# zhaoyuhsin/Edge-Guided-Near-Eye-Image-Analysis-for-Head-Mounted-Displays

Measured on AMD Instinct MI355X. Metric: eye-frames/sec (320x240): inference edge+seg (value), +fit, exact fp32, and train fwd+bwd at 1 MI355X, higher is better.
Workload: dtype f32 tensors; inference products split into f16 hi/lo pairs (3 f16 MFMAs per product, 22-bit significand), f32 accumulate (`exact_fp32`: every product on the f32 MFMA); `train`: bf16 storage, f32 accumulate, f32 master weights (and an f32-storage leg)

## Files before the change

edge-guided-near-eye-image-analysis-for-head-mounted-displays_amd/bdcn_new.py:

```python
import ctypes as C

import torch
import torch.nn as nn

from . import _lib
from . import engine
from .engine import ACT_RELU, ConvLayer, Piece, PlanarPiece, Plan, VersionGuard, maxpool_out, pad8, require_cuda

import os
import types

PLANAR_IN = os.environ.get("EGNE_PLANAR_IN", "1") != "0"
SCORES_FUSED = os.environ.get("EGNE_SCORES_FUSED", "1") != "0"
MS_SIDE_STREAM = os.environ.get("EGNE_MS_SIDE", "1") != "0"
MS_SIDE_MIN_B = int(os.environ.get("EGNE_MS_SIDE_MIN_B", "8"))

_VGG = [("conv1_1", 3, 64, 1), ("conv1_2", 64, 64, 1), ("P", 2),
        ("conv2_1", 64, 128, 1), ("conv2_2", 128, 128, 1), ("P", 2),
        ("conv3_1", 128, 256, 1), ("conv3_2", 256, 256, 1), ("conv3_3", 256, 256, 1), ("P", 2),
        ("conv4_1", 256, 512, 1), ("conv4_2", 512, 512, 1), ("conv4_3", 512, 512, 1), ("P", 1),
        ("conv5_1", 512, 512, 2), ("conv5_2", 512, 512, 2), ("conv5_3", 512, 512, 2)]
_STAGES = [("1", ["1_1", "1_2"], 64), ("2", ["2_1", "2_2"], 128), ("3", ["3_1", "3_2", "3_3"], 256),
           ("4", ["4_1", "4_2", "4_3"], 512), ("5", ["5_1", "5_2", "5_3"], 512)]
_UPS = {"2": ("upsample_2", 2, 1), "3": ("upsample_4", 4, 2), "4": ("upsample_8", 8, 4), "5": ("upsample_8_5", 8, 0)}


def get_upsampling_weight(in_channels, out_channels, kernel_size):
    factor = (kernel_size + 1) // 2
    center = factor - 1 if kernel_size % 2 == 1 else factor - 0.5
    r = 1 - (torch.arange(kernel_size, dtype=torch.float64) - center).abs() / factor
    filt = r[:, None] * r[None, :]
    w = torch.zeros((in_channels, out_channels, kernel_size, kernel_size), dtype=torch.float64)
    for i in range(min(in_channels, out_channels)):
        w[i, i] = filt
    return w.float()


class VGG16_C(nn.Module):

    def __init__(self, pretrain=None, logger=None):
        super().__init__()
        for item in _VGG:
            if item[0] == "P":
                continue
            name, cin, cout, d = item
            conv = nn.Conv2d(cin, cout, 3, stride=1, padding=d, dilation=d)
            n = 9 * cout
            conv.weight.data.normal_(0, (2.0 / n) ** 0.5)
            conv.bias.data.zero_()
            setattr(self, name, conv)
        if pretrain:
            sd = torch.load(pretrain, map_location="cpu")
            own = self.state_dict()
            for k in own:
                if k in sd:
                    own[k].copy_(sd[k])


class MSBlock(nn.Module):

    def __init__(self, c_in, rate=4):
        super().__init__()
        self.rate = rate
        self.conv = nn.Conv2d(c_in, 32, 3, stride=1, padding=1)
        for i in (1, 2, 3):
            d = rate * i if rate >= 1 else 1
            setattr(self, "conv%d" % i, nn.Conv2d(32, 32, 3, stride=1, dilation=d, padding=d))
        for m in (self.conv, self.conv1, self.conv2, self.conv3):
            m.weight.data.normal_(0, 0.01)
            m.bias.data.zero_()


class BDCN(nn.Module):
    def __init__(self, pretrain=None, logger=None, rate=4):
        super().__init__()
        self.pretrain = pretrain
        self.rate = rate
        self.features = VGG16_C(pretrain, logger)
        for st, blocks, cin in _STAGES:
            for b in blocks:
                setattr(self, "msblock" + b, MSBlock(cin, rate))
                setattr(self, "conv%s_down" % b, nn.Conv2d(32, 21, (1, 1), stride=1))
            setattr(self, "score_dsn" + st, nn.Conv2d(21, 1, (1, 1), stride=1))
            setattr(self, "score_dsn%s_1" % st, nn.Conv2d(21, 1, (1, 1), stride=1))
        self.upsample_2 = nn.ConvTranspose2d(1, 1, 4, stride=2, bias=False)
        self.upsample_4 = nn.ConvTranspose2d(1, 1, 8, stride=4, bias=False)
        self.upsample_8 = nn.ConvTranspose2d(1, 1, 16, stride=8, bias=False)
        self.upsample_8_5 = nn.ConvTranspose2d(1, 1, 16, stride=8, bias=False)
        self.fuse = nn.Conv2d(10, 1, 1, stride=1)
        self._initialize_weights()
        self._plans = {}
        self.f16_products = 0
        self._events = None
        self.edge_thres = 0

    def _initialize_weights(self, logger=None):
        with torch.no_grad():
            for name, p in self.state_dict().items():
                if self.pretrain and "features" in name:
                    continue
                if "upsample" in name:
                    k = int(name.split(".")[0].split("_")[1])
                    p.copy_(get_upsampling_weight(1, 1, k * 2))
                elif "fuse" in name:
                    p.zero_() if "bias" in name else p.fill_(0.080)
                elif "bias" in name:
                    p.zero_()
                else:
                    p.normal_(0, 0.01)

    def _build(self, B, H, W, dev, only_fuse, edge_thres, f16_storage=None, split3=False):
        if f16_storage is None:
            h8, w8 = (maxpool_out(maxpool_out(maxpool_out(n, 2), 2), 2) for n in (H, W))
            if engine.PRESPLIT_TRUNK and engine.CALIBRATE and getattr(self, "_plan_products", 0) != 1 and B * h8 * w8 >= 256 * 128:
                try:
                    return self._build(B, H, W, dev, only_fuse, edge_thres, 0, True)
                except engine.NeedsFp32Storage:
                    pass
            if engine.F16_STORAGE and getattr(self, "_plan_products", 0) == 1:
                for level in ((2, 1) if engine.F16_STORAGE_DEEP else (1,)):
                    try:
                        return self._build(B, H, W, dev, only_fuse, edge_thres, level)
                    except engine.NeedsFp32Storage:
                        pass
            return self._build(B, H, W, dev, only_fuse, edge_thres, 0)
        pl = Plan(dev)
        pl.f16_storage = int(f16_storage)
        pl.split3_trunk = bool(split3)
        pl.f16_products = getattr(self, "_plan_products", 0)
        L = pl.L
        f = self.features
        x_in = pl.vec(B, 3, H, W)
        if PLANAR_IN and engine.F16X3_ENABLED and engine.C4H_MODE != "off":
            cur = PlanarPiece(x_in)
        else:
            xb = pl.buf(B, H, W, 8)
            pl.raw(L.egne_nchw_to_nhwc, (x_in.data_ptr(), B, 3, H, W, xb.data_ptr(), 8, 0, 8), "bdcn.in")
            cur = Piece(xb, 0, 3)
        ch, hh, ww = 3, H, W
        tail = _lib.BdcnTailDesc()
        tail.B, tail.H, tail.W = B, H, W
        block_of = {}
        for si, (st, blocks, cin) in enumerate(_STAGES):
            for bi, b in enumerate(blocks):
                block_of["conv" + b] = (si, bi)
        stages = {}
        side = MS_SIDE_STREAM and B >= MS_SIDE_MIN_B

        def stage_state(si, h_s, w_s):
            if si in stages:
                return stages[si]
            st, blocks, cin = _STAGES[si]
            nb = len(blocks)
            S = types.SimpleNamespace(st=st, blocks=blocks, nb=nb, h=h_s, w=w_s, ms_bufs=[], fused=None)
            S.o_buf = pl.buf(B, h_s, w_s, 32)
            S.dn = [getattr(self, "conv%s_down" % b) for b in blocks]
            S.sa, S.sb = getattr(self, "score_dsn" + st), getattr(self, "score_dsn%s_1" % st)
            S.s, S.s1 = pl.vec(B, h_s, w_s), pl.vec(B, h_s, w_s)
            S.cw, S.cc = pl.vec(nb, 2, 32), pl.vec(2)

            def refresh_scores(cw=S.cw, cc=S.cc, dn=S.dn, sa=S.sa, sb=S.sb):
                with torch.no_grad():
                    heads = torch.stack([sa.weight.detach().reshape(21), sb.weight.detach().reshape(21)])
                    for k, m in enumerate(dn):
                        cw[k].copy_(heads @ m.weight.detach().reshape(21, 32))
                    bsum = torch.stack([m.bias.detach() for m in dn]).sum(0)
                    cc.copy_(heads @ bsum + torch.cat([sa.bias.detach(), sb.bias.detach()]))
            S.refresh_scores = refresh_scores
            stages[si] = S
            return S

        def emit_block(si, bi, src, c_in, hh, ww):
            S = stage_state(si, hh, ww)
            b = S.blocks[bi]
            pl.side_default = side
            mb = getattr(self, "msblock" + b)
            l0 = ConvLayer([mb.conv.weight], [mb.conv.bias], [(c_in, pad8(c_in))], pad=(1, 1), act=ACT_RELU)
            l0.split = True
            o = Piece(S.o_buf, 0, 32)
            r = self.rate
            dil = tuple(r * i if r >= 1 else 1 for i in (1, 2, 3))
            lg = ConvLayer([mb.conv1.weight, mb.conv2.weight, mb.conv3.weight],
                           [mb.conv1.bias, mb.conv2.bias, mb.conv3.bias], [(32, 32)], pad=(1, 1), dils=dil,
                           act=ACT_RELU)
            lg.split = True
            if engine.PRESPLIT and pl.msdil_ok(lg, o, hh, ww):
                o.presplit = engine.SplitScale()
            pl.conv(l0, [src], o, B, hh, ww, name="ms%s.conv" % b)
            if not pl.last_presplit:
                o.presplit = None
            if S.fused is None:
                S.fused = SCORES_FUSED and pl.msdil_ok(lg, o, hh, ww)
                if S.fused:
                    pl.pre.append(VersionGuard([p for m in S.dn + [S.sa, S.sb] for p in (m.weight, m.bias)], S.refresh_scores))
            if S.fused:
                pl.conv(lg, [o], Piece(S.o_buf, 0, 32), B, hh, ww, residual=o, name="ms%s.dil" % b, scores=(S.cw[bi], S.cc, S.s, S.s1, bi > 0))
            else:
                msb = pl.buf(B, hh, ww, 32)
                pl.conv(lg, [o], Piece(msb, 0, 32), B, hh, ww, residual=o, name="ms%s.dil" % b)
                S.ms_bufs.append(msb)
            if bi == S.nb - 1:
                finish_stage(si, S)
            pl.side_default = False

        def finish_stage(si, S):
            st, nb, dn, sa, sb, s, s1 = S.st, S.nb, S.dn, S.sa, S.sb, S.s, S.s1
            if not S.fused:
                wd, bd = pl.vec(nb, 21, 32), pl.vec(nb, 21)
                heads = pl.vec(2, 21)
                hb = pl.vec(2)

                def refresh(wd=wd, bd=bd, heads=heads, hb=hb, dn=dn, sa=sa, sb=sb):
                    with torch.no_grad():
                        for k, m in enumerate(dn):
                            wd[k].copy_(m.weight.detach().reshape(21, 32))
                            bd[k].copy_(m.bias.detach())
                        heads[0].copy_(sa.weight.detach().reshape(21))
                        heads[1].copy_(sb.weight.detach().reshape(21))
                        hb[0:1].copy_(sa.bias.detach())
                        hb[1:2].copy_(sb.bias.detach())
                pl.pre.append(VersionGuard([p for m in dn + [sa, sb] for p in (m.weight, m.bias)], refresh))
                arr = (C.c_void_p * nb)(*[t.data_ptr() for t in S.ms_bufs])
                pl.keep.append(arr)
                pl.raw(L.egne_bdcn_stage_scores,
                       (arr, nb, 32, B * S.h * S.w, wd.data_ptr(), bd.data_ptr(), heads.data_ptr(), hb.data_ptr(),
                        heads.data_ptr() + 4 * 21, hb.data_ptr() + 4, s.data_ptr(), s1.data_ptr()), "bdcn.scores" + st)
            tail.s[si], tail.s1[si] = s.data_ptr(), s1.data_ptr()
            tail.h[si], tail.w[si] = S.h, S.w
            if st in _UPS:
                key, stride, crop = _UPS[st]
                upw = pl.vec(2 * stride, 2 * stride)
                mod = getattr(self, key)
                pl.pre.append(VersionGuard([mod.weight], lambda upw=upw, mod=mod: upw.copy_(
                    mod.weight.detach().reshape(upw.shape))))
                tail.up[si], tail.stride[si], tail.crop[si] = upw.data_ptr(), stride, crop
            else:
                tail.stride[si], tail.crop[si] = 1, 0

        pooled = None
        for idx, item in enumerate(_VGG):
            if item[0] == "P":
                s = item[1]
                ho, wo = maxpool_out(hh, s), maxpool_out(ww, s)
                if pooled is not None:
                    dst = pooled
                else:
                    c16 = getattr(cur, "f16s", None)
                    ob = (pl.buf16 if c16 is not None else pl.buf)(B, ho, wo, cur.Cp)
                    dst = Piece(ob, 0, cur.C)
                    dst.f16s = c16
                    dst.split3 = cur.split3
                    pl.maxpool2(cur, dst, B, hh, ww, s, "vgg.pool")
                cur, hh, ww, pooled = dst, ho, wo, None
                continue
            name, cin, cout, d = item
            conv = getattr(f, name)
            layer = ConvLayer([conv.weight], [conv.bias], [(cin, pad8(cin))], pad=(1, 1), dils=(d,), act=ACT_RELU)
            layer.split = cin % 32 == 0
            layer.split_c4 = cin <= 4
            h16 = (f16_storage >= 1 and name in ("conv1_1", "conv1_2")) or (f16_storage >= 2 and name[4] in "345")
            ob = (pl.buf16 if h16 else pl.buf)(B, hh, ww, cout)
            dst = Piece(ob, 0, cout)
            if h16:
                dst.f16s = engine.SplitScale()
            if split3 and name[4] in "345":
                dst.split3 = engine.SplitScale()
            nxt = _VGG[idx + 1] if idx + 1 < len(_VGG) else None
            pq = None
            if nxt is not None and nxt[0] == "P" and nxt[1] == 2:
                pq = Piece((pl.buf16 if h16 else pl.buf)(B, maxpool_out(hh, 2), maxpool_out(ww, 2), pad8(cout)), 0, cout)
                pq.f16s = dst.f16s
            pl.conv(layer, [cur], dst, B, hh, ww, name="vgg." + name, pool=pq)
            pooled = pq if pl.last_pooled else None
            cur = dst
            si, bi = block_of[name]
            emit_block(si, bi, dst, cout, hh, ww)
        pl.serial_timing = True
        pl.join_before.add(len(pl.calls))
        fw, fb = pl.vec(10), pl.vec(1)
        pl.pre.append(VersionGuard([self.fuse.weight, self.fuse.bias], lambda: (
            fw.copy_(self.fuse.weight.detach().reshape(10)), fb.copy_(self.fuse.bias.detach()))))
        tail.fuse_w, tail.fuse_b = fw.data_ptr(), fb.data_ptr()
        outs = pl.vec(11, B, 1, H, W)
        for k in range(11):
            tail.out[k] = outs[k].data_ptr() if (k == 10 or not only_fuse) else None
        tail.edge_thres = int(edge_thres)
        pl.keep.append(tail)
        pl.raw(L.egne_bdcn_tail, (C.byref(tail),), "bdcn.tail")
        pl.x_in, pl.outs = x_in, outs
        return pl

    def _plan(self, x, only_fuse, edge_thres=0):
        require_cuda(x, "BDCN input")
        for p in self.parameters():
            require_cuda(p, "BDCN parameters (call .cuda())")
            break
        B, Cc, H, W = x.shape
        if Cc != 3:
            raise ValueError("BDCN expects a 3-channel input, got %d" % Cc)
        prod = 1 if int(getattr(self, "f16_products", 0)) == 1 else 0
        key = (B, H, W, x.device, bool(only_fuse), int(edge_thres), prod)
        if key not in self._plans:
            self._plan_products = prod
            self._plans[key] = self._build(B, H, W, x.device, only_fuse, edge_thres)
        return self._plans[key]

    def forward(self, x):
        pl = self._plan(x, only_fuse=False)
        self._last_plan = pl
        pl.x_in.copy_(x.to(torch.float32))
        pl.run()
        return [pl.outs[k].clone() for k in range(11)]

    def forward_fuse(self, x, edge_thres=0):
        pl = self._plan(x, only_fuse=True, edge_thres=edge_thres)
        self._last_plan = pl
        pl.x_in.copy_(x.to(torch.float32))
        pl.run(self._events)
        return pl.outs[10].clone()

    def overflowed(self):
        pl = getattr(self, "_last_plan", None)
        return pl is not None and pl.overflowed()
```

edge-guided-near-eye-image-analysis-for-head-mounted-displays_amd/csrc/conv3x3_c4_f16.hip:

```cpp
#include "common.h"
#include "kernel_util.h"
#include "split_f16.h"

namespace {

__device__ __forceinline__ void split8(const u32x4 a, const u32x4 b, float s, h8& hi, h8& lo) {
  const f32x4 va = __builtin_bit_cast(f32x4, a), vb = __builtin_bit_cast(f32x4, b);
  const float x[8] = {va[0], va[1], va[2], va[3], vb[0], vb[1], vb[2], vb[3]};
#pragma unroll
  for (int q = 0; q < 4; ++q) {
    h2 h, l;
    egne::split2(x[2 * q], x[2 * q + 1], s, h, l);
    hi[2 * q] = h[0]; hi[2 * q + 1] = h[1];
    lo[2 * q] = l[0]; lo[2 * q + 1] = l[1];
  }
}

template <int TN>
__global__ __launch_bounds__(256) void conv3x3_c4_f16_kernel(const egne_conv_desc p, const _Float16* __restrict__ fhi,
                                                             const _Float16* __restrict__ flo, float a_scale, float out_scale,
                                                             long long M, int nblocks) {
  const int tid = threadIdx.x, lane = tid & 63, wave = tid >> 6;
  const int li = lane & 31, kq = lane >> 5;
  const egne_seg sg = p.seg[0];
  h8 wh[3][TN], wl[3][TN];
#pragma unroll
  for (int s = 0; s < 3; ++s)
#pragma unroll
    for (int tn = 0; tn < TN; ++tn) {
      wh[s][tn] = *(const h8*)(fhi + ((s * TN + tn) * 64 + lane) * 8);
      wl[s][tn] = *(const h8*)(flo + ((s * TN + tn) * 64 + lane) * 8);
    }
  const float slope = p.act == EGNE_ACT_RELU ? 0.f : (p.act == EGNE_ACT_LEAKY ? 0.01f : 1.f);
  f32x4 bias[TN][4], ps[TN][4], pt[TN][4];
#pragma unroll
  for (int tn = 0; tn < TN; ++tn)
#pragma unroll
    for (int j = 0; j < 4; ++j) {
      const int n = tn * 32 + 8 * j + 4 * kq;
      const bool nok = n < p.Cout_store;
      bias[tn][j] = (p.bias && nok) ? *(const f32x4*)(p.bias + n) : (f32x4)(0.f);
      ps[tn][j] = (p.post_scale && nok) ? *(const f32x4*)(p.post_scale + n) : (f32x4)(1.f);
      pt[tn][j] = (p.post_scale && nok) ? *(const f32x4*)(p.post_shift + n) : (f32x4)(0.f);
    }
  const int hw = p.H * p.W;
  const int ps4 = (int)sg.pix_stride * 4;
  const unsigned frame_in = (unsigned)hw * (unsigned)ps4;

  for (int blk = blockIdx.x * 4 + wave; blk < nblocks; blk += gridDim.x * 4) {
    const long long m = (long long)blk * 32 + li;
    const int b = (int)(m / hw);
    const int r = (int)(m - (long long)b * hw);
    const int y = r / p.W, x = r - y * p.W;
    const int b0 = (int)(((long long)blk * 32) / hw);
    const bool planar = sg.pix_stride == 1;
    const int fstride = planar ? hw * sg.Cp : hw * (int)sg.pix_stride;
    const long long left = ((long long)p.B - b0) * fstride * 4;
    const __amdgpu_buffer_rsrc_t rin = make_rsrc(sg.ptr + (long long)b0 * fstride, (unsigned)(left < 0x7fffffffll ? left : 0x7fffffffll));
    const int base = planar ? ((b - b0) * fstride + r) * 4 : (((b - b0) * hw + r) * (int)sg.pix_stride + sg.ch_off) * 4;
    (void)frame_in;
    f32x16 acc[TN];
#pragma unroll
    for (int tn = 0; tn < TN; ++tn) acc[tn] = (f32x16)(0.f);
    u32x4 xa[3], xb[3];
#pragma unroll
    for (int s = 0; s < 3; ++s) {
      const int t0 = 4 * s + 2 * kq, t1 = t0 + 1;
      const int dy0 = t0 / 3 - 1, dx0 = t0 % 3 - 1, dy1 = t1 / 3 - 1, dx1 = t1 % 3 - 1;
      const bool ok0 = m < M && t0 < 9 && (unsigned)(y + dy0) < (unsigned)p.H && (unsigned)(x + dx0) < (unsigned)p.W;
      const bool ok1 = m < M && t1 < 9 && (unsigned)(y + dy1) < (unsigned)p.H && (unsigned)(x + dx1) < (unsigned)p.W;
      if (planar) {
        const int o0 = ok0 ? base + (dy0 * p.W + dx0) * 4 : (int)OOB, o1 = ok1 ? base + (dy1 * p.W + dx1) * 4 : (int)OOB;
        u32x4 a = {0u, 0u, 0u, 0u}, c = {0u, 0u, 0u, 0u};
#pragma unroll
        for (int ch = 0; ch < 4; ++ch)
          if (ch < sg.Cp) {
            a[ch] = __builtin_amdgcn_raw_buffer_load_b32(rin, o0, ch * hw * 4, 0);
            c[ch] = __builtin_amdgcn_raw_buffer_load_b32(rin, o1, ch * hw * 4, 0);
          }
        xa[s] = a; xb[s] = c;
      } else {
        xa[s] = __builtin_amdgcn_raw_buffer_load_b128(rin, ok0 ? base + (dy0 * p.W + dx0) * ps4 : (int)OOB, 0, 0);
        xb[s] = __builtin_amdgcn_raw_buffer_load_b128(rin, ok1 ? base + (dy1 * p.W + dx1) * ps4 : (int)OOB, 0, 0);
      }
    }
#pragma unroll
    for (int s = 0; s < 3; ++s) {
      h8 ah, al;
      split8(xa[s], xb[s], a_scale, ah, al);
#pragma unroll
      for (int tn = 0; tn < TN; ++tn) {
        acc[tn] = __builtin_amdgcn_mfma_f32_32x32x16_f16(wh[s][tn], al, acc[tn], 0, 0, 0);
        acc[tn] = __builtin_amdgcn_mfma_f32_32x32x16_f16(wl[s][tn], ah, acc[tn], 0, 0, 0);
        acc[tn] = __builtin_amdgcn_mfma_f32_32x32x16_f16(wh[s][tn], ah, acc[tn], 0, 0, 0);
      }
    }
    const long long m0 = (long long)blk * 32;
    const long long rows = M - m0 < 32 ? M - m0 : 32;
    const bool o16 = p.out_split == 2;
    const int oesz = o16 ? 2 : 4;
    const __amdgpu_buffer_rsrc_t ro = make_rsrc((char*)p.out + m0 * p.out_pix_stride * oesz, (unsigned)(rows * p.out_pix_stride * oesz));
    bool bad = false;
#pragma unroll
    for (int tn = 0; tn < TN; ++tn)
#pragma unroll
      for (int j = 0; j < 4; ++j) {
        const int n = tn * 32 + 8 * j + 4 * kq;
        f32x4 v;
#pragma unroll
        for (int e = 0; e < 4; ++e) {
          const float t = acc[tn][4 * j + e] * out_scale + bias[tn][j][e];
          v[e] = fmaxf(t, t * slope) * ps[tn][j][e] + pt[tn][j][e];
        }
        if (tn == 0 && j == 0) bad |= egne_nonfinite(v[0]);
        if (o16) {
          const f32x2 u0 = {v[0] * p.out_split_scale, v[1] * p.out_split_scale}, u1 = {v[2] * p.out_split_scale, v[3] * p.out_split_scale};
          const h2 h0 = __builtin_convertvector(u0, h2), h1 = __builtin_convertvector(u1, h2);
          if (tn == 0 && j == 0) bad |= egne_nonfinite((float)h0[0]);
          const u32x2 two = {__builtin_bit_cast(unsigned, h0), __builtin_bit_cast(unsigned, h1)};
          __builtin_amdgcn_raw_buffer_store_b64(two, ro, n < p.Cout_store ? (li * (int)p.out_pix_stride + p.out_ch_off + n) * 2 : (int)OOB, 0, 0);
        } else
        __builtin_amdgcn_raw_buffer_store_b128(__builtin_bit_cast(u32x4, v), ro,
                                               n < p.Cout_store ? (li * (int)p.out_pix_stride + p.out_ch_off + n) * 4 : (int)OOB, 0, 0);
      }
    egne_ovf_commit(bad, p.ovf_flag);
  }
}

__global__ void pack_c4_f16_k(const float* __restrict__ w, int Cout, int Cin, int NT, float wscale, _Float16* __restrict__ hi,
                              _Float16* __restrict__ lo) {
  const int total = 3 * NT * 512;
  for (int i = blockIdx.x * blockDim.x + threadIdx.x; i < total; i += gridDim.x * blockDim.x) {
    const int j = i & 7, nn = (i >> 3) & 31, h = (i >> 8) & 1;
    const int q = i >> 9;
    const int tn = q % NT, s = q / NT;
    const int n = tn * 32 + nn, tap = 4 * s + 2 * h + (j >> 2), c = j & 3;
    const float v = (n < Cout && tap < 9 && c < Cin) ? w[((long long)n * Cin + c) * 9 + tap] * wscale : 0.f;
    const _Float16 hh = (_Float16)v;
    hi[i] = hh;
    lo[i] = (_Float16)(v - (float)hh);
  }
}

}

extern "C" int egne_pack_conv3x3_c4_weight_f16(const float* w_oihw, int Cout, int Cin, int CoutP, float wscale, void* fhi, void* flo,
                                               void* stream) {
  EGNE_REQUIRE(w_oihw && fhi && flo && Cout > 0 && Cin > 0 && Cin <= 4 && (CoutP == 32 || CoutP == 64) && Cout <= CoutP && wscale > 0.f,
               "pack_conv3x3_c4_f16: bad sizes Cout %d Cin %d CoutP %d", Cout, Cin, CoutP);
  hipLaunchKernelGGL(pack_c4_f16_k, dim3(6), dim3(256), 0, (hipStream_t)stream, w_oihw, Cout, Cin, CoutP / 32, wscale, (_Float16*)fhi,
                     (_Float16*)flo);
  return egne::check_launch("egne_pack_conv3x3_c4_weight_f16");
}

extern "C" int egne_conv3x3_smallcin_f16_fwd(const egne_conv_desc* dp, const void* fhi, const void* flo, float a_scale, float w_scale,
                                             void* stream) {
  EGNE_REQUIRE(dp && fhi && flo, "conv_smallcin_f16: null pointer");
  const egne_conv_desc& d = *dp;
  EGNE_REQUIRE(d.kh == 3 && d.kw == 3 && d.stride == 1 && d.pad_h == 1 && d.pad_w == 1 && d.pad_mode == 0 && d.ngroups == 1 &&
               d.dil[0] == 1 && d.nseg == 1 && d.Ho == d.H && d.Wo == d.W && !d.residual, "conv_smallcin_f16: geometry not supported");
  const egne_seg& g = d.seg[0];
  const bool planar = g.pix_stride == 1;
  EGNE_REQUIRE(g.ptr && !g.scale && ((uintptr_t)g.ptr & 15) == 0 &&
               (planar ? (g.Cp >= 1 && g.Cp <= 4 && g.ch_off == 0 && 2ll * d.H * d.W * g.Cp * 4 < (1ll << 31))
                       : (g.Cp >= 4 && g.ch_off % 4 == 0 && g.pix_stride % 4 == 0 && 2ll * d.H * d.W * g.pix_stride * 4 < (1ll << 31))),
               "conv_smallcin_f16: input slice");
  EGNE_REQUIRE((d.CoutP == 32 || d.CoutP == 64) && d.Cout_store <= d.CoutP && d.Cout_store % 4 == 0 && d.out && ((uintptr_t)d.out & 15) == 0 &&
               d.out_ch_off % 4 == 0 && d.out_pix_stride % 4 == 0 && d.out_ch_off + d.Cout_store <= d.out_pix_stride &&
               d.out_pix_stride * 128 < (1ll << 31) && (!d.bias || ((uintptr_t)d.bias & 15) == 0) &&
               (!d.post_scale || (((uintptr_t)d.post_scale & 15) == 0 && ((uintptr_t)d.post_shift & 15) == 0)), "conv_smallcin_f16: output");
  EGNE_REQUIRE(((uintptr_t)fhi & 15) == 0 && ((uintptr_t)flo & 15) == 0 && a_scale > 0.f && w_scale > 0.f, "conv_smallcin_f16: weights / scales");
  EGNE_REQUIRE(d.out_split == 0 || (d.out_split == 2 && d.out_split_scale > 0.f && !d.post_scale), "conv_smallcin_f16: f16 output (out_split = 2) needs a positive scale and no post affine");
  const long long M = (long long)d.B * d.H * d.W;
  const long long nb = (M + 31) / 32;
  EGNE_REQUIRE(nb < (1ll << 31), "conv_smallcin_f16: too many pixels");
  long long gx = (nb + 3) / 4;
  if (gx > 256 * 8) gx = 256 * 8;
  const float os = 1.0f / (a_scale * w_scale);
  hipStream_t st = (hipStream_t)stream;
  if (d.CoutP == 32)
    hipLaunchKernelGGL((conv3x3_c4_f16_kernel<1>), dim3((unsigned)gx), dim3(256), 0, st, d, (const _Float16*)fhi, (const _Float16*)flo, a_scale, os,
                       M, (int)nb);
  else
    hipLaunchKernelGGL((conv3x3_c4_f16_kernel<2>), dim3((unsigned)gx), dim3(256), 0, st, d, (const _Float16*)fhi, (const _Float16*)flo, a_scale, os,
                       M, (int)nb);
  return egne::check_launch("egne_conv3x3_smallcin_f16_fwd");
}
```

edge-guided-near-eye-image-analysis-for-head-mounted-displays_amd/csrc/conv3x3_rw_f16.hip:

```cpp
#include "common.h"
#include "kernel_util.h"
#include "split_f16.h"
#include <cstdlib>
#include <type_traits>

namespace {
__device__ int g_wdbg = 0;
__device__ unsigned long long g_wstamps[256 * 8 * 4];

constexpr int TW = 32, TH = 8, HWd = TW + 2, HHd = TH + 2, NPX = HHd * HWd;
constexpr int IMGH = 2 * NPX * 32;
constexpr int WCH = 9 * 2 * 2 * 512;
constexpr int NI = (NPX * 8 + 255) / 256;

template <int KCH, int NP = 3, bool F16IN = false, int SH = 0>
__global__ __launch_bounds__(512)
void conv3x3_rw_kernel(const egne_conv_desc p, const _Float16* __restrict__ fhi, const _Float16* __restrict__ flo, float a_scale,
                       float out_scale, int tiles_x, int tiles_y, int ntiles, int ncb, int nrun) {
  egne::dyn_scales(p.dyn_scale, a_scale, out_scale);
  extern __shared__ __attribute__((aligned(16))) _Float16 ldsh[];
  _Float16* const lw = ldsh + 2 * IMGH;

  const int dbg = g_wdbg;
  unsigned long long t_work = 0, t_wait = 0, t_hand = 0, t_last = 0;
  auto stamp = [&](unsigned long long& accum) {
    if (dbg & 64) {
      asm volatile("s_waitcnt lgkmcnt(0)" ::: "memory");
      const unsigned long long t = __builtin_amdgcn_s_memtime();
      accum += t - t_last; t_last = t;
    }
  };
  const int tid = threadIdx.x, lane = tid & 63;
  const int wave = __builtin_amdgcn_readfirstlane(tid >> 6);
  const int li = lane & 31, lh = lane >> 5;
  const int H = p.H, W = p.W;
  const egne_seg sg = p.seg[0];

  const int xcd = blockIdx.x & 7, q = blockIdx.x >> 3;
  const int wpx = ((int)gridDim.x >> 3) / nrun;
  if (q >= wpx * nrun) return;
  const int cb = q % nrun, worker = (q / nrun) * 8 + xcd, nworkers = wpx * 8;
  auto tile_at = [&](int i) { return worker + i * nworkers; };
  struct Tile { int b, y0, x0; };
  auto decode = [&](int t) {
    Tile r;
    const int tx = t % tiles_x; t /= tiles_x;
    const int ty = t % tiles_y; t /= tiles_y;
    r.b = t; r.y0 = ty * TH; r.x0 = tx * TW;
    return r;
  };
  int ntl = 0;
  while (tile_at(ntl) < ntiles) ++ntl;
  constexpr bool STREAM = KCH == 0;
  const int nk = STREAM ? p.Ktot / 32 : KCH;
  const int nmine = ntl * nk;
  const int nloop = (nmine + 1) & ~1;

  const int KT16 = nk * 2;
  if constexpr (!STREAM) {
    for (int it = tid; it < KCH * 9 * 2 * 2 * 64; it += 512) {
      const int l = it & 63, hl = (it >> 6) & 1, ks = (it >> 7) & 1, r = it >> 8, tap = r % 9, ch = r / 9;
      const long long src = (((long long)tap * KT16 + ch * 2 + ks) * ncb + cb) * 512 + l * 8;
      *(u32x4*)&lw[(long long)it * 8] = *(const u32x4*)((hl ? flo : fhi) + src);
    }
  }
  __syncthreads();

  if (wave < 4) {
    constexpr int NPC = F16IN ? 4 : 8, PGS = 256 / NPC, CPP = 32 / NPC, ESZ = F16IN ? 2 : 4, NQ = (NPX * NPC + 255) / 256;
    const int piece = tid & (NPC - 1), pg = tid / NPC;
    const float slope_in = sg.act_in == EGNE_ACT_RELU ? 0.f : (sg.act_in == EGNE_ACT_LEAKY ? 0.01f : 1.f);
    const int lofs = F16IN ? pg * 32 + ((piece ^ ((pg >> 1) & 3)) << 3) : pg * 32 + (((piece >> 1) ^ ((pg >> 1) & 3)) << 3) + ((piece & 1) << 2);
    u32x4 st[2][NQ];
    int rel[NQ];
#pragma unroll
    for (int I = 0; I < NQ; ++I) {
      const int px = pg + PGS * I, hy = px / HWd, hx = px - hy * HWd;
      rel[I] = px < NPX ? (((hy - 1) * W + hx - 1) * (int)sg.pix_stride + sg.ch_off + piece * CPP) * ESZ : (int)OOB;
    }
    struct Job { Tile t; int ch; };
    auto job_at = [&](int j) { Job r; r.t = decode(tile_at(j / nk)); r.ch = j % nk; return r; };
    auto issue1 = [&](const Job& jb, bool on, auto bc, auto ic) {
      constexpr int BUF = decltype(bc)::value, I = decltype(ic)::value;
      const Tile& tl = jb.t;
      const __amdgpu_buffer_rsrc_t r = make_rsrc((const char*)sg.ptr + (long long)tl.b * H * W * sg.pix_stride * ESZ, (unsigned)H * W * (unsigned)sg.pix_stride * (unsigned)ESZ);
      const int c0 = jb.ch * 32 + piece * CPP;
      int off;
      if (tl.x0 >= 1 && tl.x0 + TW + 1 <= W) {
        const int sbase = ((tl.y0 * W + tl.x0) * (int)sg.pix_stride + jb.ch * 32) * ESZ;
        off = (on && c0 < sg.Cp && rel[I] != (int)OOB) ? rel[I] + sbase : (int)OOB;
      } else {
        int pq = pg;
        asm volatile("" : "+v"(pq));
        const int px = pq + PGS * I;
        const int hy = px / HWd, hx = px - hy * HWd;
        const int y = tl.y0 - 1 + hy, x = tl.x0 - 1 + hx;
        const bool ok = on && c0 < sg.Cp && px < NPX && (unsigned)y < (unsigned)H && (unsigned)x < (unsigned)W;
        off = ok ? ((y * W + x) * (int)sg.pix_stride + sg.ch_off + c0) * ESZ : (int)OOB;
      }
      st[BUF][I] = __builtin_amdgcn_raw_buffer_load_b128(r, off, 0, 0);
    };
    f32x4 asc[2] = {{1.f, 1.f, 1.f, 1.f}, {1.f, 1.f, 1.f, 1.f}}, ash[2] = {{0.f, 0.f, 0.f, 0.f}, {0.f, 0.f, 0.f, 0.f}};
    auto load_aff = [&](const Job& jb, auto bc) {
      constexpr int BUF = decltype(bc)::value;
      if (sg.scale && nmine > 0) {
        const int c0 = jb.ch * 32 + piece * 4;
        const float* zs = c0 < sg.Cp ? sg.scale + (long long)jb.t.b * sg.Cp + c0 : egne_zero_page;
        const float* zh = c0 < sg.Cp ? sg.shift + (long long)jb.t.b * sg.Cp + c0 : egne_zero_page;
        asc[BUF] = *(const f32x4*)zs;
        ash[BUF] = *(const f32x4*)zh;
      }
    };
    auto convert1 = [&](const Job& jb, _Float16* img, auto bc, auto ic) {
      constexpr int BUF = decltype(bc)::value, I = decltype(ic)::value;
      const int px = pg + PGS * I;
      if constexpr (F16IN) {
        if (I < NQ - 1 || px < NPX) *(u32x4*)&img[lofs + 32 * PGS * I] = st[BUF][I];
        return;
      }
      if (I < NQ - 1 || px < NPX) {
        f32x4 v = __builtin_bit_cast(f32x4, st[BUF][I]);
        if (sg.scale) {
          const int hy = px / HWd, hx = px - hy * HWd;
          const int y = jb.t.y0 - 1 + hy, x = jb.t.x0 - 1 + hx;
#pragma unroll
          for (int e = 0; e < 4; ++e) {
            const float t = v[e] * asc[BUF][e] + ash[BUF][e];
            v[e] = fmaxf(t, t * slope_in);
          }
          if (!((unsigned)y < (unsigned)H && (unsigned)x < (unsigned)W)) v = (f32x4)(0.f);
        }
        const int o = lofs + 32 * PGS * I;
        if constexpr (NP == 1) {
          float t0, t1, t2, t3;
          asm("v_mul_f32_e32 %0, %1, %2" : "=v"(t0) : "s"(a_scale), "v"(v[0]));
          asm("v_mul_f32_e32 %0, %1, %2" : "=v"(t1) : "s"(a_scale), "v"(v[1]));
          asm("v_mul_f32_e32 %0, %1, %2" : "=v"(t2) : "s"(a_scale), "v"(v[2]));
          asm("v_mul_f32_e32 %0, %1, %2" : "=v"(t3) : "s"(a_scale), "v"(v[3]));
          const egne::sp_f32x2 u0 = {t0, t1}, u1 = {t2, t3};
          const h2 h0 = __builtin_convertvector(u0, h2), h1 = __builtin_convertvector(u1, h2);
          const h4 hi = {h0[0], h0[1], h1[0], h1[1]};
          *(h4*)&img[o] = hi;
        } else {
        h2 h0, h1, l0, l1;
        egne::split2(v[0], v[1], a_scale, h0, l0);
        egne::split2(v[2], v[3], a_scale, h1, l1);
        const h4 hi = {h0[0], h0[1], h1[0], h1[1]}, lo = {l0[0], l0[1], l1[0], l1[1]};
        *(h4*)&img[o] = hi;
        *(h4*)&img[NPX * 32 + o] = lo;
        }
      }
    };
    u32x4 wreg[STREAM ? 9 : 1];
    const unsigned wbytes = 9u * (unsigned)KT16 * (unsigned)ncb * 1024u;
    const __amdgpu_buffer_rsrc_t rwh = make_rsrc(fhi, wbytes), rwl = make_rsrc(flo, wbytes);
    auto w_issue = [&](int ch, bool on) {
#pragma unroll
      for (int i = 0; i < (STREAM ? 9 : 0); ++i) {
        const int it = tid + 256 * i, l = it & 63, hl = (it >> 6) & 1, ks = (it >> 7) & 1, tap = it >> 8;
        const int off = on ? ((((tap * KT16 + ch * 2 + ks) * ncb + cb) * 512 + l * 8) * 2) : (int)OOB;
        wreg[i] = hl ? __builtin_amdgcn_raw_buffer_load_b128(rwl, off, 0, 0) : __builtin_amdgcn_raw_buffer_load_b128(rwh, off, 0, 0);
      }
    };
    auto w_store = [&](int parity) {
#pragma unroll
      for (int i = 0; i < (STREAM ? 9 : 0); ++i) *(u32x4*)&lw[parity * WCH + (tid + 256 * i) * 8] = wreg[i];
    };
    auto step = [&](int s, auto bc) {
      constexpr int BUF = decltype(bc)::value;
      const bool c_on = s + 1 < nmine, i_on = s + 3 < nmine;
      const Job jc = job_at(c_on ? s + 1 : 0), ji = job_at(i_on ? s + 3 : 0);
      if constexpr (STREAM) {
        w_store((s + 1) & 1);
        w_issue(job_at(s + 2 < nmine ? s + 2 : 0).ch, s + 2 < nmine);
      }
      load_aff(job_at(s + 2 < nmine ? s + 2 : 0), std::integral_constant<int, BUF ^ 1>{});
      _Float16* img = ldsh + ((s + 1) & 1) * IMGH;
      [&]<int... Is>(std::integer_sequence<int, Is...>) {
        (([&] {
          if (c_on) convert1(jc, img, bc, std::integral_constant<int, Is>{});
          issue1(ji, i_on, bc, std::integral_constant<int, Is>{});
        }()), ...);
      }(std::make_integer_sequence<int, NQ>{});
    };
    using B0 = std::integral_constant<int, 0>;
    using B1 = std::integral_constant<int, 1>;
    {
      const Job j0 = job_at(0), j1 = job_at(nmine > 1 ? 1 : 0), j2 = job_at(nmine > 2 ? 2 : 0);
      if constexpr (STREAM) {
        w_issue(j0.ch, nmine > 0);
        w_store(0);
        w_issue(j1.ch, nmine > 1);
      }
      load_aff(j0, B0{});
      load_aff(j1, B1{});
      [&]<int... Is>(std::integer_sequence<int, Is...>) {
        (issue1(j0, nmine > 0, B0{}, std::integral_constant<int, Is>{}), ...);
        (issue1(j1, nmine > 1, B1{}, std::integral_constant<int, Is>{}), ...);
      }(std::make_integer_sequence<int, NQ>{});
      [&]<int... Is>(std::integer_sequence<int, Is...>) {
        (([&] {
          if (nmine > 0) convert1(j0, ldsh, B0{}, std::integral_constant<int, Is>{});
          issue1(j2, nmine > 2, B0{}, std::integral_constant<int, Is>{});
        }()), ...);
      }(std::make_integer_sequence<int, NQ>{});
    }
    lds_barrier();
    t_last = __builtin_amdgcn_s_memtime();
    for (int s = 0; s < nloop; s += 2) {
      step(s, B1{});
      stamp(t_work); lds_barrier(); stamp(t_wait);
      step(s + 1, B0{});
      stamp(t_work); lds_barrier(); stamp(t_wait);
    }
  } else if constexpr (SH != 0) {
    constexpr bool GEN = SH == 1;
    const int cw = wave - 4, row0 = cw * 2;
    const int l15 = lane & 15, kg = lane >> 4;
    const bool o16 = GEN && NP == 1 && p.out_split == 2;
    const bool split_on = SH == 4 || (GEN && !o16 && p.out_split != 0);
    const bool pool_on = SH == 3 || (GEN && p.pool_out != nullptr);
    const bool full_epi = SH == 5 || (GEN && (p.post_scale != nullptr || p.residual != nullptr));
    const int oesz = o16 ? 2 : 4;
    const unsigned frame_out = (unsigned)H * W * (unsigned)p.out_pix_stride * (unsigned)oesz;
    const unsigned frame_res = (unsigned)H * W * (unsigned)p.res_pix_stride * 4u;
    const int Hp = (H + 1) >> 1, Wp = (W + 1) >> 1;
    const unsigned frame_pool = (unsigned)Hp * Wp * (unsigned)p.pool_pix_stride * (unsigned)oesz;
    const float slope_out = p.act == EGNE_ACT_RELU ? 0.f : (p.act == EGNE_ACT_LEAKY ? 0.01f : 1.f);
    f32x4 b4[2];
    bool jok[2];
#pragma unroll
    for (int nh = 0; nh < 2; ++nh) {
      const int n = cb * 32 + nh * 16 + 4 * kg;
      b4[nh] = p.bias ? *(const f32x4*)(p.bias + n) : (f32x4)(0.f);
      jok[nh] = n < p.Cout_store;
    }
    int aofs[9][2][2];
#pragma unroll
    for (int tap = 0; tap < 9; ++tap)
#pragma unroll
      for (int tm = 0; tm < 2; ++tm)
#pragma unroll
        for (int ph = 0; ph < 2; ++ph) {
          const int qq = (row0 + tm + tap / 3) * HWd + ph * 16 + l15 + tap % 3;
          aofs[tap][tm][ph] = qq * 32 + ((kg ^ ((qq >> 1) & 3)) << 3);
        }
    const int wl = (kg >> 1) * 1024 + ((kg & 1) * 32 + l15) * 8;
    int xl[2], xlp[2], lco[2], lcr[2], lcp[2];
#pragma unroll
    for (int ph = 0; ph < 2; ++ph) {
      xl[ph] = ph * 16 + l15;
      xlp[ph] = (l15 & 1) ? 0x40000000 : xl[ph];
      lco[ph] = (xl[ph] * (int)p.out_pix_stride + p.out_ch_off + cb * 32 + 4 * kg) * oesz;
      lcr[ph] = (xl[ph] * (int)p.res_pix_stride + p.res_ch_off + cb * 32 + 4 * kg) * 4;
      lcp[ph] = ((xl[ph] >> 1) * (int)p.pool_pix_stride + p.pool_ch_off + cb * 32 + 4 * kg) * oesz;
    }
    f32x4 R[2][2][2][2];
#pragma unroll
    for (int a = 0; a < 16; ++a) (&R[0][0][0][0])[a] = (f32x4)(0.f);
    __amdgpu_buffer_rsrc_t rout = make_rsrc(p.out, 0u), rres = make_rsrc(nullptr, 0u), rpo = make_rsrc(nullptr, 0u);
    int wlim[2] = {0, 0}, sbo[2] = {0, 0}, sbr[2] = {0, 0}, wlim_p = 0, x1lim = 0, sbp = 0;
    bool y1 = false;
    bool have_prev = false;
    unsigned ovf_m = 0u, ovf_h = 0u;
    int tvo = (int)OOB, tvr = (int)OOB, poff = (int)OOB;
    auto epi = [&](auto qc, auto gc) {
      constexpr int Q = decltype(qc)::value, Gi = decltype(gc)::value, nh = Gi & 1, ph = (Gi >> 1) & 1, tm = Gi >> 2;
      if constexpr (tm == 0) {
        if (pool_on) {
          const bool x1 = xl[ph] < x1lim;
          if constexpr (nh == 0) poff = xlp[ph] < wlim_p ? lcp[ph] + sbp : (int)OOB;
          f32x4 v;
#pragma unroll
          for (int e = 0; e < 4; ++e) {
            float m = R[Q][0][ph][nh][e];
            m = y1 ? fmaxf(m, R[Q][1][ph][nh][e]) : m;
            const float qn = __builtin_bit_cast(float, __builtin_amdgcn_update_dpp(0, __builtin_bit_cast(int, m), 0xB1, 0xf, 0xf, false));
            m = x1 ? fmaxf(m, qn) : m;
            const float t = m * out_scale + b4[nh][e];
            v[e] = fmaxf(t, t * slope_out);
          }
          if (o16) {
            const egne::sp_f32x2 u0 = {v[0] * p.out_split_scale, v[1] * p.out_split_scale}, u1 = {v[2] * p.out_split_scale, v[3] * p.out_split_scale};
            const h2 h0 = __builtin_convertvector(u0, h2), h1 = __builtin_convertvector(u1, h2);
            const u32x2 two = {__builtin_bit_cast(unsigned, h0), __builtin_bit_cast(unsigned, h1)};
            __builtin_amdgcn_raw_buffer_store_b64(two, rpo, jok[nh] ? poff : (int)OOB, nh * 32, 0);
          } else {
            __builtin_amdgcn_raw_buffer_store_b128(__builtin_bit_cast(u32x4, v), rpo, jok[nh] ? poff : (int)OOB, nh * 64, 0);
          }
        }
      }
      if constexpr (nh == 0) {
        const bool okp = xl[ph] < wlim[tm];
        tvo = okp ? lco[ph] + sbo[tm] : (int)OOB;
        if (full_epi) tvr = okp ? lcr[ph] + sbr[tm] : (int)OOB;
      }
      f32x4 v;
#pragma unroll
      for (int e = 0; e < 4; ++e) {
        const float t = R[Q][tm][ph][nh][e] * out_scale + b4[nh][e];
        v[e] = fmaxf(t, t * slope_out);
      }
      if (full_epi) {
        const int n = cb * 32 + nh * 16 + 4 * kg;
        if (p.post_scale) {
          const f32x4 ps = *(const f32x4*)(p.post_scale + n), pt = *(const f32x4*)(p.post_shift + n);
#pragma unroll
          for (int e = 0; e < 4; ++e) v[e] = v[e] * ps[e] + pt[e];
        }
        if (p.residual) {
          const f32x4 rv = __builtin_bit_cast(f32x4, __builtin_amdgcn_raw_buffer_load_b128(rres, jok[nh] ? tvr : (int)OOB, nh * 64, 0));
#pragma unroll
          for (int e = 0; e < 4; ++e) v[e] += rv[e];
        }
      }
      if constexpr (nh == 0) ovf_m = max(ovf_m, __builtin_bit_cast(unsigned, v[0]) & 0x7fffffffu);
      if (o16) {
        const egne::sp_f32x2 u0 = {v[0] * p.out_split_scale, v[1] * p.out_split_scale}, u1 = {v[2] * p.out_split_scale, v[3] * p.out_split_scale};
        const h2 h0 = __builtin_convertvector(u0, h2), h1 = __builtin_convertvector(u1, h2);
        if constexpr (nh == 0) ovf_h = max(ovf_h, __builtin_bit_cast(unsigned, h0) & 0x7fffu);
        const u32x2 two = {__builtin_bit_cast(unsigned, h0), __builtin_bit_cast(unsigned, h1)};
        __builtin_amdgcn_raw_buffer_store_b64(two, rout, jok[nh] ? tvo : (int)OOB, nh * 32, 0);
      } else if (split_on) {
        h2 h0, h1, l0, l1;
        egne::split2(v[0], v[1], p.out_split_scale, h0, l0);
        egne::split2(v[2], v[3], p.out_split_scale, h1, l1);
        const u32x4 pk = {__builtin_bit_cast(unsigned, h0), __builtin_bit_cast(unsigned, h1), __builtin_bit_cast(unsigned, l0), __builtin_bit_cast(unsigned, l1)};
        R[Q][tm][ph][nh] = __builtin_bit_cast(f32x4, pk);
        if constexpr (nh == 1) {
          const u32x4 p0 = __builtin_bit_cast(u32x4, R[Q][tm][ph][0]), p1 = __builtin_bit_cast(u32x4, R[Q][tm][ph][1]);
          const u32x4 hi = {p0[0], p0[1], p1[0], p1[1]}, lo = {p0[2], p0[3], p1[2], p1[3]};
          __builtin_amdgcn_raw_buffer_store_b128(hi, rout, tvo, 0, 0);
          if constexpr (NP == 3) __builtin_amdgcn_raw_buffer_store_b128(lo, rout, tvo, 64, 0);
        }
      } else {
        __builtin_amdgcn_raw_buffer_store_b128(__builtin_bit_cast(u32x4, v), rout, jok[nh] ? tvo : (int)OOB, nh * 64, 0);
      }
    };
    const int d_tx = nworkers % tiles_x, d_ty = (nworkers / tiles_x) % tiles_y, d_b = (nworkers / tiles_x) / tiles_y;
    int tx = worker % tiles_x, ty = (worker / tiles_x) % tiles_y, tb = (worker / tiles_x) / tiles_y;
    int s = 0;
    auto job = [&](auto pc, auto fc, int ch) {
      constexpr int P = decltype(pc)::value;
      constexpr bool FIRST = decltype(fc)::value;
      const _Float16* Thi = ldsh + (s & 1) * IMGH;
      const _Float16* Tlo = Thi + NPX * 32;
      const _Float16* wb = lw + (STREAM ? (s & 1) : ch) * WCH + wl;
      h8 wh[2][2], wo[2][2], ah[2][2][2], al[2][2][2];
      auto fetch = [&](auto tc) {
        constexpr int T = decltype(tc)::value, Bq = T & 1;
#pragma unroll
        for (int nh = 0; nh < 2; ++nh) {
          wh[Bq][nh] = *(const h8*)&wb[T * 2048 + nh * 128];
          if constexpr (NP == 3) wo[Bq][nh] = *(const h8*)&wb[T * 2048 + 512 + nh * 128];
        }
#pragma unroll
        for (int tm = 0; tm < 2; ++tm)
#pragma unroll
          for (int ph = 0; ph < 2; ++ph) {
            ah[Bq][tm][ph] = *(const h8*)&Thi[aofs[T][tm][ph]];
            if constexpr (NP == 3) al[Bq][tm][ph] = *(const h8*)&Tlo[aofs[T][tm][ph]];
          }
      };
      fetch(std::integral_constant<int, 0>{});
      [&]<int... Ts>(std::integer_sequence<int, Ts...>) {
        (([&] {
          constexpr int t = Ts, Bq = t & 1;
          __builtin_amdgcn_sched_barrier(0);
          if constexpr (t + 1 < 9) fetch(std::integral_constant<int, t + 1>{});
          if constexpr (FIRST && t < 8) epi(std::integral_constant<int, P ^ 1>{}, std::integral_constant<int, t>{});
#pragma unroll
          for (int tm = 0; tm < 2; ++tm)
#pragma unroll
            for (int ph = 0; ph < 2; ++ph)
#pragma unroll
              for (int nh = 0; nh < 2; ++nh) {
                f32x4 c = R[P][tm][ph][nh];
                if constexpr (FIRST && t == 0) c = (f32x4)(0.f);
                if constexpr (NP == 3) {
                  c = __builtin_amdgcn_mfma_f32_16x16x32_f16(wh[Bq][nh], al[Bq][tm][ph], c, 0, 0, 0);
                  c = __builtin_amdgcn_mfma_f32_16x16x32_f16(wo[Bq][nh], ah[Bq][tm][ph], c, 0, 0, 0);
                }
                c = __builtin_amdgcn_mfma_f32_16x16x32_f16(wh[Bq][nh], ah[Bq][tm][ph], c, 0, 0, 0);
                R[P][tm][ph][nh] = c;
              }
          constexpr int NM = NP == 3 ? 24 : 8, ND = t + 1 < 9 ? (NP == 3 ? 12 : 6) : 0, NV = FIRST && SH == 3 && t < 4 ? 4 : 3;
          [&]<int... Ms>(std::integer_sequence<int, Ms...>) {
            (([&] {
              __builtin_amdgcn_sched_group_barrier(0x8, 1, 0);
              if constexpr (Ms < ND) __builtin_amdgcn_sched_group_barrier(0x100, 1, 0);
              __builtin_amdgcn_sched_group_barrier(0x2, NV, 0);
              if constexpr (FIRST && Ms >= NM - 3) __builtin_amdgcn_sched_group_barrier(0x40, 1, 0);
            }()), ...);
          }(std::make_integer_sequence<int, NM>{});
        }()), ...);
      }(std::make_integer_sequence<int, 9>{});
      __builtin_amdgcn_sched_barrier(0);
      ++s;
      stamp(t_work); lds_barrier(); stamp(t_wait);
    };
    auto tile = [&](auto pc) {
      job(pc, std::true_type{}, 0);
      for (int ch = 1; ch < nk; ++ch) job(pc, std::false_type{}, ch);
      const int py = ty * TH + row0, px = tx * TW;
#pragma unroll
      for (int tm = 0; tm < 2; ++tm) {
        const bool in = py + tm < H;
        wlim[tm] = in ? W - px : 0;
        sbo[tm] = in ? ((py + tm) * W + px) * (int)p.out_pix_stride * oesz : 0;
        if (full_epi) sbr[tm] = in ? ((py + tm) * W + px) * (int)p.res_pix_stride * 4 : 0;
      }
      if (pool_on) {
        y1 = py + 1 < H; x1lim = W - px - 1; wlim_p = wlim[0];
        sbp = py < H ? ((py >> 1) * Wp + (px >> 1)) * (int)p.pool_pix_stride * oesz : 0;
      }
      rout = make_rsrc((char*)p.out + (long long)tb * H * W * p.out_pix_stride * oesz, frame_out);
      if (full_epi) rres = make_rsrc(p.residual ? p.residual + (long long)tb * H * W * p.res_pix_stride : nullptr, p.residual ? frame_res : 0u);
      if (pool_on) rpo = make_rsrc((char*)p.pool_out + (long long)tb * Hp * Wp * p.pool_pix_stride * oesz, frame_pool);
      if (!have_prev) ovf_m = ovf_h = 0u;
      have_prev = true;
      tx += d_tx;
      int c = tx >= tiles_x ? 1 : 0;
      tx -= c ? tiles_x : 0;
      ty += d_ty + c;
      c = ty >= tiles_y ? 1 : 0;
      ty -= c ? tiles_y : 0;
      tb += d_b + c;
    };
    using P0 = std::integral_constant<int, 0>;
    using P1 = std::integral_constant<int, 1>;
    lds_barrier();
    t_last = __builtin_amdgcn_s_memtime();
    for (int i = 0; i < ntl; i += 2) {
      tile(P0{});
      if (i + 1 < ntl) tile(P1{});
    }
    if (nmine & 1) { stamp(t_work); lds_barrier(); stamp(t_wait); }
    stamp(t_work);
    if (have_prev) {
      auto flush = [&](auto qc) {
        [&]<int... Gs>(std::integer_sequence<int, Gs...>) { (epi(qc, std::integral_constant<int, Gs>{}), ...); }(std::make_integer_sequence<int, 8>{});
      };
      if (ntl & 1) flush(P0{}); else flush(P1{});
    }
    stamp(t_hand);
    const bool ovf_bad = egne_nonfinite(__builtin_bit_cast(float, ovf_m)) || egne_nonfinite((float)__builtin_bit_cast(_Float16, (unsigned short)ovf_h));
    egne_ovf_commit(ovf_bad, p.ovf_flag);
  } else {
    const int cw = wave - 4, row0 = cw * 2;
    const int l15 = lane & 15, kg = lane >> 4;
    const bool o16 = NP == 1 && p.out_split == 2;
    const int oesz = o16 ? 2 : 4;
    const unsigned frame_out = (unsigned)H * W * (unsigned)p.out_pix_stride * (unsigned)oesz;
    const unsigned frame_res = (unsigned)H * W * (unsigned)p.res_pix_stride * 4u;
    const float slope_out = p.act == EGNE_ACT_RELU ? 0.f : (p.act == EGNE_ACT_LEAKY ? 0.01f : 1.f);
    const bool full_epi = p.post_scale != nullptr || p.residual != nullptr;
    f32x4 b4[2];
    bool jok[2];
#pragma unroll
    for (int nh = 0; nh < 2; ++nh) {
      const int n = cb * 32 + nh * 16 + 4 * kg;
      b4[nh] = p.bias ? *(const f32x4*)(p.bias + n) : (f32x4)(0.f);
      jok[nh] = n < p.Cout_store;
    }
    int aofs[9][2][2];
#pragma unroll
    for (int tap = 0; tap < 9; ++tap)
#pragma unroll
      for (int tm = 0; tm < 2; ++tm)
#pragma unroll
        for (int ph = 0; ph < 2; ++ph) {
          const int qq = (row0 + tm + tap / 3) * HWd + ph * 16 + l15 + tap % 3;
          aofs[tap][tm][ph] = qq * 32 + ((kg ^ ((qq >> 1) & 3)) << 3);
        }
    const int wl = (kg >> 1) * 1024 + ((kg & 1) * 32 + l15) * 8;
    f32x4 acc[2][2][2], prev[2][2][2];
#pragma unroll
    for (int a = 0; a < 8; ++a) { (&acc[0][0][0])[a] = (f32x4)(0.f); (&prev[0][0][0])[a] = (f32x4)(0.f); }
    __amdgpu_buffer_rsrc_t rout = make_rsrc(p.out, 0u), rres = make_rsrc(nullptr, 0u);
    int tvo[2][2], tvr[2][2];
#pragma unroll
    for (int a = 0; a < 4; ++a) { (&tvo[0][0])[a] = (int)OOB; (&tvr[0][0])[a] = (int)OOB; }
    bool ovf_bad = false;
    auto finish_group = [&](auto gc) {
      constexpr int Gi = decltype(gc)::value, nh = Gi & 1, ph = (Gi >> 1) & 1, tm = Gi >> 2;
      f32x4 v;
#pragma unroll
      for (int e = 0; e < 4; ++e) {
        const float t = prev[tm][ph][nh][e] * out_scale + b4[nh][e];
        v[e] = fmaxf(t, t * slope_out);
      }
      if (full_epi) {
        const int n = cb * 32 + nh * 16 + 4 * kg;
        if (p.post_scale) {
          const f32x4 ps = *(const f32x4*)(p.post_scale + n), pt = *(const f32x4*)(p.post_shift + n);
#pragma unroll
          for (int e = 0; e < 4; ++e) v[e] = v[e] * ps[e] + pt[e];
        }
        if (p.residual) {
          const f32x4 rv = __builtin_bit_cast(f32x4, __builtin_amdgcn_raw_buffer_load_b128(rres, jok[nh] ? tvr[tm][ph] : (int)OOB, nh * 64, 0));
#pragma unroll
          for (int e = 0; e < 4; ++e) v[e] += rv[e];
        }
      }
      if constexpr (nh == 0) ovf_bad |= egne_nonfinite(v[0]);
      if (o16) {
        const egne::sp_f32x2 u0 = {v[0] * p.out_split_scale, v[1] * p.out_split_scale}, u1 = {v[2] * p.out_split_scale, v[3] * p.out_split_scale};
        const h2 h0 = __builtin_convertvector(u0, h2), h1 = __builtin_convertvector(u1, h2);
        if constexpr (nh == 0) ovf_bad |= egne_nonfinite((float)h0[0]);
        v[0] = __builtin_bit_cast(float, h0);
        v[1] = __builtin_bit_cast(float, h1);
      } else if (p.out_split) {
        h2 h0, h1, l0, l1;
        egne::split2(v[0], v[1], p.out_split_scale, h0, l0);
        egne::split2(v[2], v[3], p.out_split_scale, h1, l1);
        const u32x4 pk = {__builtin_bit_cast(unsigned, h0), __builtin_bit_cast(unsigned, h1), __builtin_bit_cast(unsigned, l0), __builtin_bit_cast(unsigned, l1)};
        v = __builtin_bit_cast(f32x4, pk);
      }
      prev[tm][ph][nh] = v;
    };
    auto store_group = [&](auto gc) {
      constexpr int Gi = decltype(gc)::value, nh = Gi & 1, ph = (Gi >> 1) & 1, tm = Gi >> 2;
      if (o16) {
        const u32x4 pk = __builtin_bit_cast(u32x4, prev[tm][ph][nh]);
        const u32x2 two = {pk[0], pk[1]};
        __builtin_amdgcn_raw_buffer_store_b64(two, rout, jok[nh] ? tvo[tm][ph] : (int)OOB, nh * 32, 0);
      } else if (p.out_split) {
        if constexpr (nh == 1) {
          const u32x4 p0 = __builtin_bit_cast(u32x4, prev[tm][ph][0]), p1 = __builtin_bit_cast(u32x4, prev[tm][ph][1]);
          const u32x4 hi = {p0[0], p0[1], p1[0], p1[1]}, lo = {p0[2], p0[3], p1[2], p1[3]};
          __builtin_amdgcn_raw_buffer_store_b128(hi, rout, tvo[tm][ph], 0, 0);
          if constexpr (NP == 3) __builtin_amdgcn_raw_buffer_store_b128(lo, rout, tvo[tm][ph], 64, 0);
        }
      } else {
        __builtin_amdgcn_raw_buffer_store_b128(__builtin_bit_cast(u32x4, prev[tm][ph][nh]), rout, jok[nh] ? tvo[tm][ph] : (int)OOB, nh * 64, 0);
      }
    };
    bool have_prev = false;
    lds_barrier();
    t_last = __builtin_amdgcn_s_memtime();
    for (int s = 0; s < nloop; ++s) {
      if (s < nmine) {
        const int ch = s % nk;
        const Tile tl = decode(tile_at(s / nk));
        const _Float16* Thi = ldsh + (s & 1) * IMGH;
        const _Float16* Tlo = Thi + NPX * 32;
        const _Float16* wb = lw + (STREAM ? (s & 1) : ch) * WCH + wl;
        if (ch == 0) {
#pragma unroll
          for (int a = 0; a < 8; ++a) (&acc[0][0][0])[a] = (f32x4)(0.f);
        }
        h8 wh[2][2], wo[2][2], ah[2][2][2], al[2][2][2];
        auto fetch = [&](auto tc) {
          constexpr int T = decltype(tc)::value, Bq = T & 1;
#pragma unroll
          for (int nh = 0; nh < 2; ++nh) {
            wh[Bq][nh] = *(const h8*)&wb[T * 2048 + nh * 128];
            if constexpr (NP == 3) wo[Bq][nh] = *(const h8*)&wb[T * 2048 + 512 + nh * 128];
          }
#pragma unroll
          for (int tm = 0; tm < 2; ++tm)
#pragma unroll
            for (int ph = 0; ph < 2; ++ph) {
              ah[Bq][tm][ph] = *(const h8*)&Thi[aofs[T][tm][ph]];
              if constexpr (NP == 3) al[Bq][tm][ph] = *(const h8*)&Tlo[aofs[T][tm][ph]];
            }
        };
        fetch(std::integral_constant<int, 0>{});
        [&]<int... Ts>(std::integer_sequence<int, Ts...>) {
          (([&] {
            constexpr int t = Ts, Bq = t & 1;
            if constexpr (t + 1 < 9) fetch(std::integral_constant<int, t + 1>{});
            if constexpr (t < 8) { if (ch == 0 && have_prev) store_group(std::integral_constant<int, t>{}); }
            __builtin_amdgcn_sched_barrier(0);
#pragma unroll
            for (int tm = 0; tm < 2; ++tm)
#pragma unroll
              for (int ph = 0; ph < 2; ++ph)
#pragma unroll
                for (int nh = 0; nh < 2; ++nh) {
                  f32x4& c = acc[tm][ph][nh];
                  if constexpr (NP == 3) {
                    c = __builtin_amdgcn_mfma_f32_16x16x32_f16(wh[Bq][nh], al[Bq][tm][ph], c, 0, 0, 0);
                    c = __builtin_amdgcn_mfma_f32_16x16x32_f16(wo[Bq][nh], ah[Bq][tm][ph], c, 0, 0, 0);
                  }
                  c = __builtin_amdgcn_mfma_f32_16x16x32_f16(wh[Bq][nh], ah[Bq][tm][ph], c, 0, 0, 0);
                }
            __builtin_amdgcn_sched_barrier(0);
          }()), ...);
        }(std::make_integer_sequence<int, 9>{});
        if (ch == nk - 1) {
          stamp(t_work);
          const int y = tl.y0 + row0;
          if (p.pool_out) {
            const int Hp = (H + 1) >> 1, Wp = (W + 1) >> 1;
            const __amdgpu_buffer_rsrc_t rpo = make_rsrc((char*)p.pool_out + (long long)tl.b * Hp * Wp * p.pool_pix_stride * oesz,
                                                         (unsigned)Hp * Wp * (unsigned)p.pool_pix_stride * (unsigned)oesz);
            const bool y1 = y + 1 < H;
#pragma unroll
            for (int ph = 0; ph < 2; ++ph) {
              const int x = tl.x0 + ph * 16 + l15;
              const bool x1 = x + 1 < W;
              const int poff = (!(l15 & 1) && x < W && y < H) ? (((y >> 1) * Wp + (x >> 1)) * (int)p.pool_pix_stride + p.pool_ch_off + cb * 32 + 4 * kg) * oesz : (int)OOB;
#pragma unroll
              for (int nh = 0; nh < 2; ++nh) {
                f32x4 v;
#pragma unroll
                for (int e = 0; e < 4; ++e) {
                  float m = acc[0][ph][nh][e];
                  if (y1) m = fmaxf(m, acc[1][ph][nh][e]);
                  const float qn = __builtin_bit_cast(float, __builtin_amdgcn_update_dpp(0, __builtin_bit_cast(int, m), 0xB1, 0xf, 0xf, false));
                  if (x1) m = fmaxf(m, qn);
                  const float t = m * out_scale + b4[nh][e];
                  v[e] = fmaxf(t, t * slope_out);
                }
                if (o16) {
                  const egne::sp_f32x2 u0 = {v[0] * p.out_split_scale, v[1] * p.out_split_scale}, u1 = {v[2] * p.out_split_scale, v[3] * p.out_split_scale};
                  const h2 h0 = __builtin_convertvector(u0, h2), h1 = __builtin_convertvector(u1, h2);
                  const u32x2 two = {__builtin_bit_cast(unsigned, h0), __builtin_bit_cast(unsigned, h1)};
                  __builtin_amdgcn_raw_buffer_store_b64(two, rpo, jok[nh] ? poff : (int)OOB, nh * 32, 0);
                } else {
                  __builtin_amdgcn_raw_buffer_store_b128(__builtin_bit_cast(u32x4, v), rpo, jok[nh] ? poff : (int)OOB, nh * 64, 0);
                }
              }
            }
          }
#pragma unroll
          for (int a = 0; a < 8; ++a) (&prev[0][0][0])[a] = (&acc[0][0][0])[a];
          rout = make_rsrc((char*)p.out + (long long)tl.b * H * W * p.out_pix_stride * oesz, frame_out);
          rres = make_rsrc(p.residual ? p.residual + (long long)tl.b * H * W * p.res_pix_stride : nullptr, p.residual ? frame_res : 0u);
#pragma unroll
          for (int tm = 0; tm < 2; ++tm)
#pragma unroll
            for (int ph = 0; ph < 2; ++ph) {
              const int yy = y + tm, x = tl.x0 + ph * 16 + l15;
              const bool okp = yy < H && x < W;
              tvo[tm][ph] = okp ? ((yy * W + x) * (int)p.out_pix_stride + p.out_ch_off + cb * 32 + 4 * kg) * oesz : (int)OOB;
              tvr[tm][ph] = okp ? ((yy * W + x) * (int)p.res_pix_stride + p.res_ch_off + cb * 32 + 4 * kg) * 4 : (int)OOB;
            }
          [&]<int... Gs>(std::integer_sequence<int, Gs...>) { (finish_group(std::integral_constant<int, Gs>{}), ...); }(std::make_integer_sequence<int, 8>{});
          have_prev = true;
          stamp(t_hand);
        }
      }
      stamp(t_work); lds_barrier(); stamp(t_wait);
    }
    if (have_prev)
      [&]<int... Gs>(std::integer_sequence<int, Gs...>) { (store_group(std::integral_constant<int, Gs>{}), ...); }(std::make_integer_sequence<int, 8>{});
    egne_ovf_commit(ovf_bad, p.ovf_flag);
  }
  if ((dbg & 64) && lane == 0) {
    unsigned long long* o = g_wstamps + ((long long)blockIdx.x * 8 + wave) * 4;
    o[0] = t_work + t_hand; o[1] = t_wait; o[2] = nmine; o[3] = t_hand;
  }
}

template <int KCH, int NP, bool F16IN, int SH>
int launch_rw_form(const egne_conv_desc& d, const _Float16* fhi, const _Float16* flo, float a_scale, float os, hipStream_t st);

template <int KCH, int NP = 3, bool F16IN = false>
int launch_rw(const egne_conv_desc& d, const _Float16* fhi, const _Float16* flo, float a_scale, float os, hipStream_t st) {
  const char* e = getenv("EGNE_RW_SHADOW");
  if (e && e[0] == '0') return launch_rw_form<KCH, NP, F16IN, 0>(d, fhi, flo, a_scale, os, st);
  if constexpr (NP == 3) {
    if ((d.post_scale || d.residual) && d.pool_out) return launch_rw_form<KCH, NP, F16IN, 0>(d, fhi, flo, a_scale, os, st);
    if (d.post_scale || d.residual) return launch_rw_form<KCH, NP, F16IN, 5>(d, fhi, flo, a_scale, os, st);
    if (d.pool_out) return launch_rw_form<KCH, NP, F16IN, 3>(d, fhi, flo, a_scale, os, st);
    if (d.out_split) return launch_rw_form<KCH, NP, F16IN, 4>(d, fhi, flo, a_scale, os, st);
    return launch_rw_form<KCH, NP, F16IN, 2>(d, fhi, flo, a_scale, os, st);
  } else {
    return launch_rw_form<KCH, NP, F16IN, 1>(d, fhi, flo, a_scale, os, st);
  }
}

template <int KCH, int NP, bool F16IN, int SH>
int launch_rw_form(const egne_conv_desc& d, const _Float16* fhi, const _Float16* flo, float a_scale, float os, hipStream_t st) {
  const int tiles_x = (d.W + TW - 1) / TW, tiles_y = (d.H + TH - 1) / TH;
  const int ntiles = tiles_x * tiles_y * d.B, ncb = d.CoutP / 32, nrun = (d.Cout_store + 31) / 32;
  constexpr size_t lds = ((size_t)2 * IMGH + (size_t)(KCH == 0 ? 2 : KCH) * WCH) * sizeof(_Float16);
  static_assert(lds <= 163840, "LDS budget");
  if (!egne::raise_lds((const void*)conv3x3_rw_kernel<KCH, NP, F16IN, SH>, lds)) return egne::fail(EGNE_ERR_LAUNCH, "conv3x3_rw: cannot raise the dynamic LDS limit to %zu", lds);
  hipLaunchKernelGGL((conv3x3_rw_kernel<KCH, NP, F16IN, SH>), dim3(256), dim3(512), lds, st, d, fhi, flo, a_scale, os, tiles_x, tiles_y, ntiles, ncb, nrun);
  return egne::check_launch("egne_conv3x3_rw_f16_fwd");
}

}

extern "C" int egne_conv3x3_rw_f16_fwd(const egne_conv_desc* dp, const void* fhi, const void* flo, float a_scale, float w_scale,
                                       void* stream) {
  EGNE_REQUIRE(dp && fhi && flo, "conv3x3_rw: null pointer");
  const egne_conv_desc& d = *dp;
  EGNE_REQUIRE(d.kh == 3 && d.kw == 3 && d.stride == 1 && d.pad_mode == 0 && d.ngroups == 1 && d.nseg == 1 && d.pad_h == 1 &&
               d.pad_w == 1 && d.dil[0] == 1 && d.Ho == d.H && d.Wo == d.W && !d.stats_ws, "conv3x3_rw: geometry / options not supported");
  const egne_seg& g = d.seg[0];
  EGNE_REQUIRE(g.ptr && g.Cp % 8 == 0 && (g.Cp + 31) / 32 * 32 == d.Ktot && d.Ktot >= 32 && d.Ktot <= 1024 && g.ch_off % 4 == 0 &&
               g.pix_stride % 4 == 0 && ((uintptr_t)g.ptr & 15) == 0 && (g.scale == nullptr) == (g.shift == nullptr), "conv3x3_rw: input slice");
  EGNE_REQUIRE(d.CoutP % 32 == 0 && d.CoutP <= 256 && d.Cout_store >= 8 && d.Cout_store <= d.CoutP && d.Cout_store % 8 == 0 && d.out &&
               ((uintptr_t)d.out & 15) == 0 && d.out_pix_stride % 4 == 0 && d.out_ch_off % 4 == 0 &&
               d.out_ch_off + d.Cout_store <= d.out_pix_stride && (!d.bias || ((uintptr_t)d.bias & 15) == 0), "conv3x3_rw: output");
  EGNE_REQUIRE(!d.residual || (((uintptr_t)d.residual & 15) == 0 && d.res_pix_stride % 4 == 0 && d.res_ch_off % 4 == 0), "conv3x3_rw: residual alignment");
  EGNE_REQUIRE(!d.post_scale || (((uintptr_t)d.post_scale & 15) == 0 && ((uintptr_t)d.post_shift & 15) == 0), "conv3x3_rw: post affine alignment");
  EGNE_REQUIRE(!d.pool_out || (((uintptr_t)d.pool_out & 15) == 0 && d.pool_pix_stride % 4 == 0 && d.pool_ch_off % 4 == 0 && !d.post_scale &&
                                d.pool_ch_off + d.Cout_store <= d.pool_pix_stride &&
                                (long long)((d.H + 1) / 2) * ((d.W + 1) / 2) * d.pool_pix_stride * 4 < (1ll << 31)), "conv3x3_rw: pooled output");
  EGNE_REQUIRE(((uintptr_t)fhi & 15) == 0 && ((uintptr_t)flo & 15) == 0 && a_scale > 0.f && w_scale > 0.f, "conv3x3_rw: weights / scales");
  EGNE_REQUIRE(d.out_split != 1 || (d.out_split_scale > 0.f && d.Cout_store % 32 == 0 && d.out_ch_off % 32 == 0 && !d.pool_out && !d.post_scale && !d.residual),
               "conv3x3_rw: split-pair output needs whole 32-channel blocks, a positive scale and no pooled / post-affine / residual options");
  EGNE_REQUIRE(d.out_split == 0 || d.out_split == 1 || (d.out_split == 2 && d.f16_products == 1 && d.out_split_scale > 0.f && !d.post_scale && !d.residual),
               "conv3x3_rw: f16 output (out_split = 2) needs f16_products = 1, a positive scale and no post-affine / residual options");
  const bool in16 = g.presplit == 2;
  EGNE_REQUIRE(g.presplit == 0 || (in16 && d.f16_products == 1 && !g.scale && g.ch_off % 8 == 0 && g.pix_stride % 8 == 0 &&
                                   (long long)d.H * d.W * g.pix_stride * 2 < (1ll << 31)),
               "conv3x3_rw: an f16 input slice (presplit = 2) needs f16_products = 1, no fused affine and 16-byte aligned pixels");
  EGNE_REQUIRE((long long)d.H * d.W * g.pix_stride * 4 < (1ll << 31) && (long long)d.H * d.W * d.out_pix_stride * 4 < (1ll << 31) &&
               (!d.residual || (long long)d.H * d.W * d.res_pix_stride * 4 < (1ll << 31)), "conv3x3_rw: frame too large for 32-bit byte offsets");
  const float os = 1.0f / (a_scale * w_scale);
  hipStream_t st = (hipStream_t)stream;
  const _Float16 *h = (const _Float16*)fhi, *l = (const _Float16*)flo;
  if (d.f16_products == 1 && in16) {
    if (d.Ktot == 32) return launch_rw<1, 1, true>(d, h, l, a_scale, os, st);
    if (d.Ktot == 64) return launch_rw<2, 1, true>(d, h, l, a_scale, os, st);
    return launch_rw<0, 1, true>(d, h, l, a_scale, os, st);
  }
  if (d.f16_products == 1) {
    if (d.Ktot == 32) return launch_rw<1, 1>(d, h, l, a_scale, os, st);
    if (d.Ktot == 64) return launch_rw<2, 1>(d, h, l, a_scale, os, st);
    return launch_rw<0, 1>(d, h, l, a_scale, os, st);
  }
  if (d.Ktot == 32) return launch_rw<1>(d, h, l, a_scale, os, st);
  if (d.Ktot == 64) return launch_rw<2>(d, h, l, a_scale, os, st);
  return launch_rw<0>(d, h, l, a_scale, os, st);
}

extern "C" int egne_rw_debug(int dbg, void* out_stamps) {
  if (hipMemcpyToSymbol(HIP_SYMBOL(g_wdbg), &dbg, sizeof(int)) != hipSuccess) return -2;
  if (out_stamps && hipMemcpyFromSymbol(out_stamps, HIP_SYMBOL(g_wstamps), sizeof(unsigned long long) * 256 * 8 * 4) != hipSuccess) return -2;
  return 0;
}
```

edge-guided-near-eye-image-analysis-for-head-mounted-displays_amd/engine.py:

```python
import collections
import ctypes as C
import types

import torch

from . import _lib
from ._lib import ACT_LEAKY, ACT_NONE, ACT_RELU


import os

HALO_ENABLED = os.environ.get("EGNE_HALO", "1") != "0"
F16X3_ENABLED = os.environ.get("EGNE_F16X3", "1") != "0"
HALO_F16_MAX_COUTP = int(os.environ.get("EGNE_HALO_F16_MAX_COUTP", "256"))
LATTICE_ENABLED = os.environ.get("EGNE_LATTICE", "1") != "0"
LAYER_BYTES = {}
TDPOOL_FUSED = os.environ.get("EGNE_TDPOOL_FUSED", "1") != "0"
TDPOOL_STATS_UNITS = 32768
HALO_POOL = os.environ.get("EGNE_HALO_POOL", "1") != "0"
POOL_FUSED = os.environ.get("EGNE_POOL_FUSED", "1") != "0"
RW_MIN_W = int(os.environ.get("EGNE_RW_MIN_W", "120"))
RW_MAX_COUTP = int(os.environ.get("EGNE_RW_MAX_COUTP", "32"))
RW_MAX_CP = int(os.environ.get("EGNE_RW_MAX_CP", "512"))
RW_ENABLED = os.environ.get("EGNE_RW", "1") != "0"
RS_ENABLED = os.environ.get("EGNE_RS", "1") != "0"
RS_MIN_W = int(os.environ.get("EGNE_RS_MIN_W", "60"))
RS_MIN_W_F16 = int(os.environ.get("EGNE_RS_MIN_W_F16", "30"))
RW_MIN_W_F16 = int(os.environ.get("EGNE_RW_MIN_W_F16", "30"))
NARROW_F32 = os.environ.get("EGNE_NARROW_F32", "1") != "0"
TAIL16_HALO = os.environ.get("EGNE_TAIL16_HALO", "1") != "0"
MSDIL_ENABLED = os.environ.get("EGNE_MSDIL", "1") != "0"
LATTICE_MIN_W = int(os.environ.get("EGNE_LATTICE_MIN_W", "20"))
S1X1_ENABLED = os.environ.get("EGNE_S1X1", "1") != "0"
MS1X1_ENABLED = os.environ.get("EGNE_MS1X1", "1") != "0"
C4H_MODE = os.environ.get("EGNE_C4H", "wide")
MS1X1_MIN_PIX = int(os.environ.get("EGNE_MS1X1_MIN_PIX", "30000"))
BIG_ENABLED = os.environ.get("EGNE_BIG", "1") != "0"
SMALL_ENABLED = os.environ.get("EGNE_SMALL", "1") != "0"
BIG_MIN_COUT = int(os.environ.get("EGNE_BIG_MIN_COUT", "256"))
BIG_MIN_CIN = int(os.environ.get("EGNE_BIG_MIN_CIN", "64"))
BIG_SPLIT_TAIL = os.environ.get("EGNE_BIG_SPLIT_TAIL", "1") != "0"
BIG_CUS = 256
BIG1_ENABLED = os.environ.get("EGNE_BIG1", "1") != "0"
WINDOW_NAME = os.environ.get("EGNE_FIT_WINDOW", "enc.b3.conv1")
WINDOW_HOOKS = []
EVENT_KINDS = None
S1X1_MIN_PIX = int(os.environ.get("EGNE_S1X1_MIN_PIX", "100000"))
HALO_F16_ENABLED = os.environ.get("EGNE_HALO_F16", "1") != "0"
ESF_SPLIT = os.environ.get("EGNE_ESF_SPLIT", "1") != "0"
ZERO_SKIP = os.environ.get("EGNE_ZERO_SKIP", "1") != "0"
FIRST_WRITER = os.environ.get("EGNE_FIRST_WRITER", "1") != "0"
PAIR_BIAS = os.environ.get("EGNE_PAIR_BIAS", "1") != "0"
ZERO_AHEAD = os.environ.get("EGNE_ZERO_AHEAD", "1") != "0"
PAIR_BIAS_SIDE = os.environ.get("EGNE_PAIR_BIAS_SIDE", "1") != "0"
MERGE_DGRAD = os.environ.get("EGNE_MERGE_DGRAD", "1") != "0"
WGRAD_SPLIT = os.environ.get("EGNE_WGRAD_SPLIT", "1") != "0"
WGRAD_SIDE_STREAM = os.environ.get("EGNE_WGRAD_SIDE", "1") != "0"
WSCALE_EVERY = int(os.environ.get("EGNE_WSCALE_EVERY", "16"))
TRAIN_SPLIT = os.environ.get("EGNE_TRAIN_SPLIT", "1") != "0"
F16X3_ASCALE = float(os.environ.get("EGNE_F16X3_ASCALE", "16"))
STATS_FUSED = os.environ.get("EGNE_STATS_FUSED", "1") != "0"
STATS_FUSED_BF16 = os.environ.get("EGNE_STATS_FUSED_BF16", "1") != "0"
FUSE_1X1 = os.environ.get("EGNE_FUSE_1X1", "1") != "0"
FUSE_1X1_MIN_W = int(os.environ.get("EGNE_FUSE_1X1_MIN_W", "60"))
FUSE_C4 = os.environ.get("EGNE_FUSE_C4", "1") != "0"
C1V = os.environ.get("EGNE_C1V", "1") != "0"
CALIBRATE = os.environ.get("EGNE_CALIBRATE", "1") != "0"
RECAL_EVERY = int(os.environ.get("EGNE_RECAL_EVERY", "1024"))
CHECK_DISPATCH = os.environ.get("EGNE_CHECK_DISPATCH", "0") != "0"
DISPATCH_LOG = []
OVF_CHECK = os.environ.get("EGNE_OVF_CHECK", "1") != "0"
SMALLCIN_ENABLED = os.environ.get("EGNE_SMALLCIN", "1") != "0"
HALO_MIN_W = int(os.environ.get("EGNE_HALO_MIN_W", "30"))
HALO_TALL = os.environ.get("EGNE_SHALO_TALL", "1") != "0"
HALO_F16_MIN_W = int(os.environ.get("EGNE_HALO_F16_MIN_W", "30"))
HALO_F16_MIN_W_NARROW = int(os.environ.get("EGNE_HALO_F16_MIN_W_NARROW", "30"))
HALO_MAX_COUTP = int(os.environ.get("EGNE_HALO_MAX_COUTP", "128"))
NORM_FUSE = os.environ.get("EGNE_NORM_FUSE", "1") != "0"
PREFIX_ACC = os.environ.get("EGNE_PREFIX_ACC", "1") != "0"
BN_ACT_FUSE = os.environ.get("EGNE_BN_ACT_FUSE", "1") != "0"
MULTI_DGRAD = os.environ.get("EGNE_MULTI_DGRAD", "1") != "0"
MASK_ON_WRITE = os.environ.get("EGNE_MASK_ON_WRITE", "1") != "0"
MULTI_SINGLE = os.environ.get("EGNE_MULTI_SINGLE", "1") != "0"
MASK3_ON_WRITE = os.environ.get("EGNE_MASK3_ON_WRITE", "1") != "0"
BF16_FAST1X1 = os.environ.get("EGNE_BF16_FAST1X1", "1") != "0"
BF16_DGRAD_PACK = os.environ.get("EGNE_BF16_DGRAD_PACK", "1") != "0"
BF16_NARROW = os.environ.get("EGNE_BF16_NARROW", "1") != "0"
BF16_FAST3X3 = os.environ.get("EGNE_BF16_FAST3X3", "1") != "0"


def pad8(c):
    return (int(c) + 7) // 8 * 8


def pad32(c):
    return (int(c) + 31) // 32 * 32


def _ptr(t, elem_off=0):
    return t.data_ptr() + 4 * int(elem_off)


class Piece:

    __slots__ = ("buf", "off", "C", "Cp", "n0", "scale", "shift", "act_in", "nograd", "presplit", "norm_fuse", "f16s", "split3")

    def __init__(self, buf, off, C_, Cp=None, n0=0):
        self.buf, self.off, self.C, self.Cp, self.n0 = buf, int(off), int(C_), int(Cp or pad8(C_)), int(n0)
        self.scale = self.shift = None
        self.act_in = ACT_NONE
        self.nograd = False
        self.presplit = None
        self.f16s = None
        self.split3 = None
        self.norm_fuse = False
        assert self.off % 4 == 0 and self.Cp % 8 == 0 and self.off + self.Cp <= buf.shape[-1]

    @property
    def stride(self):
        return self.buf.shape[-1]

    @property
    def ptr(self):
        hw = self.buf.shape[1] * self.buf.shape[2]
        return self.buf.data_ptr() + self.buf.element_size() * (self.n0 * hw * self.stride)

    def with_norm(self, scale, shift, act_in=ACT_NONE):
        p = Piece(self.buf, self.off, self.C, self.Cp, self.n0)
        p.scale, p.shift, p.act_in, p.nograd, p.norm_fuse = scale, shift, act_in, self.nograd, self.norm_fuse
        return p

    def samples(self, n0):
        return Piece(self.buf, self.off, self.C, self.Cp, n0)


class SplitScale:

    def __init__(self):
        self.value = F16X3_ASCALE


class NeedsFp32Storage(Exception):
    """Plan.conv: a slice held as f16 (Piece.f16s) met a kernel that neither writes nor reads that storage -- the plan builder falls
    back to fp32 tensors (bdcn_new.BDCN._build)."""


F16_STORAGE = os.environ.get("EGNE_F16_STORAGE", "1") != "0"
F16_STORAGE_DEEP = os.environ.get("EGNE_F16_STORAGE_DEEP", "1") != "0"
PRESPLIT_TRUNK = os.environ.get("EGNE_PRESPLIT_TRUNK", "1") != "0"
PRESPLIT = os.environ.get("EGNE_PRESPLIT", "1") != "0"
SPLIT_PAIR_PERM = torch.tensor([16 * ((p >> 2) & 1) + 4 * (p >> 3) + (p & 3) for p in range(32)])


class ConvLayer:

    def __init__(self, weights, biases, in_layout, stride=1, pad=(0, 0), dils=(1,), act=ACT_NONE, pad_mode=0,
                 kernel_hw=None, cout_pad=None):
        self.weights = list(weights)
        self.biases = list(biases) if biases is not None else None
        self.in_layout = [(int(c), int(cp)) for c, cp in in_layout]
        w0 = self.weights[0]
        self.Cout = w0.shape[0]
        self.Cin = sum(c for c, _ in self.in_layout)
        self.kh, self.kw = kernel_hw if kernel_hw else (w0.shape[2], w0.shape[3])
        assert w0.numel() == self.Cout * self.Cin * self.kh * self.kw, (tuple(w0.shape), self.Cin, self.kh, self.kw)
        self.stride, self.pad, self.dils, self.act, self.pad_mode = stride, pad, tuple(dils), act, pad_mode
        self.Ktot = sum(cp for _, cp in self.in_layout)
        self.CoutP = pad32(self.Cout)
        self.Cout_store = cout_pad if cout_pad else pad8(self.Cout)
        self.G = len(self.weights)
        self.wp = None
        self.wf = None
        self.split = False
        self.need_split = False
        self.need_sfrag = False
        self.halo_wide96 = False
        self.need_c4h = False
        self.c4hi = self.c4lo = None
        self.need_m1 = False
        self.m1hi = self.m1lo = None
        self.need_big = False
        self.wimg = None
        self.need_big1 = False
        self.wimg1 = None
        self.need_bfrag = False
        self.bfrag = None
        self.split1 = False
        self.need_s1 = False
        self.s1hi = self.s1lo = None
        self.whi = self.wlo = None
        self.fhi = self.flo = None
        self.w_scale = 1.0
        self.need_flat = False
        self.need_frag = False
        self.bp = None
        self._versions = None
        self.post = None
        self.k_perm = None

    def _kinv(self, dev):
        k, c0 = [], 0
        for c, cp in self.in_layout:
            k += list(range(c0, c0 + c)) + [-1] * (cp - c)
            c0 += c
        return torch.tensor(k, dtype=torch.int32, device=dev)

    def ensure_packed(self, dev):
        vers = tuple(w._version for w in self.weights) + tuple(
            (b._version if b is not None else -1) for b in (self.biases or [])) + (id(getattr(self, "k_perm", None)),)
        have = (getattr(self, "w40", None) is not None or not getattr(self, "need_c4", False)) and ((self.wp is not None or not self.need_flat) and (self.wf is not None or not self.need_frag)
                and (self.whi is not None or not self.need_split) and (self._sfrag_ready() or not self.need_sfrag)
                and (self.s1hi is not None or not self.need_s1) and (self.wimg is not None or not self.need_big) and (self.wimg1 is not None or not self.need_big1)
                and (self.m1hi is not None or not self.need_m1) and (self.c4hi is not None or not self.need_c4h)
                and (self.bfrag is not None or not self.need_bfrag)
                and (getattr(self, "b1frag", None) is not None or not getattr(self, "need_b1", False)))
        if self.bp is not None and have and vers == self._versions and self.bp.device == dev:
            if self.need_sfrag:
                self._sfrag_select()
            return False
        L = _lib.lib()
        T = self.kh * self.kw
        n = self.G * T * self.CoutP * self.Ktot
        if self.bp is None or self.bp.device != dev:
            self.bp = torch.zeros(self.G * self.CoutP, dtype=torch.float32, device=dev)
            self.kinv = self._kinv(dev)
            self.wp = self.wf = None
        if self.need_flat and self.wp is None:
            self.wp = torch.empty(n, dtype=torch.float32, device=dev)
        if self.need_frag and self.wf is None:
            self.wf = torch.empty(n, dtype=torch.float32, device=dev)
        st = _lib.stream_ptr()
        for g, w in enumerate(self.weights):
            wd = w.detach()
            assert wd.is_cuda and wd.dtype == torch.float32
            wd = wd.contiguous()
            for need, buf, fn in ((self.need_flat, self.wp, L.egne_pack_conv_weight),
                                  (self.need_frag, self.wf, L.egne_pack_conv_weight_frag)):
                if need:
                    _lib.check(fn(wd.data_ptr(), self.Cout, self.Cin, self.kh, self.kw, self.kinv.data_ptr(),
                                  self.CoutP, self.Ktot, _ptr(buf, g * T * self.CoutP * self.Ktot), st), "pack_conv_weight")
            if self.biases is not None and self.biases[g] is not None:
                self.bp[g * self.CoutP: g * self.CoutP + self.Cout].copy_(self.biases[g].detach())
        if getattr(self, "need_c4", False):
            n32 = 32 if self.Cout_store <= 32 else 64
            if getattr(self, "w40", None) is None:
                self.w40 = torch.zeros(n32, 40, dtype=torch.float32, device=dev)
            wd = self.weights[0].detach()
            self.w40.zero_()
            self.w40[:self.Cout, :36].view(self.Cout, 9, 4)[:, :, :self.Cin].copy_(wd.permute(0, 2, 3, 1).reshape(self.Cout, 9, self.Cin))
        if self.need_s1:
            import math
            wd = self.weights[0].detach().contiguous()
            mx = float(wd.abs().max())
            self.w_scale1 = 2.0 ** math.floor(math.log2(2048.0 / mx)) if mx > 0 else 1.0
            if self.s1hi is None:
                kmap, c0 = [], 0
                for c, cp in self.in_layout:
                    for g in range((cp + 15) // 16):
                        for h in range(2):
                            for j in range(8):
                                ch = 16 * g + (4 * h + j if j < 4 else 8 + 4 * h + j - 4)
                                kmap.append(c0 + ch if ch < c else -1)
                    c0 += c
                self.s1_G = len(kmap) // 16
                self.s1_kmap = torch.tensor(kmap, dtype=torch.int32, device=dev)
                self.s1hi = torch.empty(self.s1_G * self.CoutP * 16, dtype=torch.float16, device=dev)
                self.s1lo = torch.empty_like(self.s1hi)
            _lib.check(L.egne_pack_conv1x1_weight_f16(wd.data_ptr(), self.Cout, self.Cin, self.s1_kmap.data_ptr(), self.s1_G, self.CoutP,
                                                      self.w_scale1, self.s1hi.data_ptr(), self.s1lo.data_ptr(), st), "pack_conv1x1_f16")
        if self.need_c4h:
            import math
            wd = self.weights[0].detach().contiguous()
            mx = float(wd.abs().max())
            self.w_scale_c4 = 2.0 ** math.floor(math.log2(2048.0 / mx)) if mx > 0 else 1.0
            self.c4_coutp = 32 if self.Cout_store <= 32 else 64
            if self.c4hi is None:
                self.c4hi = torch.empty(3 * self.c4_coutp * 16, dtype=torch.float16, device=dev)
                self.c4lo = torch.empty_like(self.c4hi)
            _lib.check(L.egne_pack_conv3x3_c4_weight_f16(wd.data_ptr(), self.Cout, self.Cin, self.c4_coutp, self.w_scale_c4,
                                                         self.c4hi.data_ptr(), self.c4lo.data_ptr(), st), "pack_conv3x3_c4_f16")
        if self.need_m1:
            import math
            wd = self.weights[0].detach().contiguous()
            mx = float(wd.abs().max())
            self.w_scale_m1 = 2.0 ** math.floor(math.log2(2048.0 / mx)) if mx > 0 else 1.0
            if self.m1hi is None:
                kmap, c0 = [], 0
                for c, cp in self.in_layout:
                    kmap += list(range(c0, c0 + c)) + [-1] * (pad32(cp) - c)
                    c0 += c
                self.m1_ktot = len(kmap)
                self.m1_coutp = (self.Cout + 63) // 64 * 64
                self.m1_kmap = torch.tensor(kmap, dtype=torch.int32, device=dev)
                self.m1hi = torch.empty(self.m1_coutp * self.m1_ktot, dtype=torch.float16, device=dev)
                self.m1lo = torch.empty_like(self.m1hi)
            _lib.check(L.egne_pack_conv1x1_weight_f16x2_map(wd.data_ptr(), self.Cout, self.Cin, self.m1_kmap.data_ptr(), self.m1_coutp,
                                                            self.m1_ktot, self.w_scale_m1, self.m1hi.data_ptr(), self.m1lo.data_ptr(), st),
                       "pack_conv1x1_f16x2_map")
        if self.need_big:
            import math
            wd = self.weights[0].detach().contiguous()
            mx = float(wd.abs().max())
            self.w_scale_big = 2.0 ** math.floor(math.log2(2048.0 / mx)) if mx > 0 else 1.0
            bn = 256 if self.Cout % 256 == 0 else 128
            self.big_bn, self.big_coutp = bn, (self.Cout + bn - 1) // bn * bn
            kts = pad32(self.Ktot)
            if self.wimg is None:
                self.wimg = torch.empty(self.big_coutp * kts * T * 2, dtype=torch.float16, device=dev)
            _lib.check(L.egne_pack_conv_weight_f16img(wd.data_ptr(), self.Cout, self.Cin, self.kh, self.kw, bn, kts, self.w_scale_big,
                                                      self.wimg.data_ptr(), st), "pack_f16img")
            if self.need_big1:
                if self.wimg1 is None:
                    self.wimg1 = torch.empty(self.big_coutp * kts * T, dtype=torch.float16, device=dev)
                _lib.check(L.egne_pack_conv_weight_f16img1(wd.data_ptr(), self.Cout, self.Cin, self.kh, self.kw, bn, kts, self.w_scale_big,
                                                           self.wimg1.data_ptr(), st), "pack_f16img1")
        if getattr(self, "need_b1", False):
            _pack_b1(self, dev, st)
        if self.need_bfrag:
            wd = self.weights[0].detach().contiguous()
            kts = pad32(self.Ktot)
            if self.bfrag is None:
                self.bfrag = torch.empty(T * self.CoutP * kts, dtype=torch.bfloat16, device=dev)
            _lib.check(L.egne_pack_conv_weight_bf16frag(wd.data_ptr(), self.Cout, self.Cin, self.kh, self.kw, self.CoutP, kts,
                                                        self.bfrag.data_ptr(), st), "pack_bf16frag")
        if self.need_split or self.need_sfrag:
            import math
            ws = [w.detach().contiguous() for w in self.weights]
            if getattr(self, "k_perm", None) is not None:
                ws = [w[:, self.k_perm.to(w.device)].contiguous() for w in ws]
            age = getattr(self, "_ws_age", 0)
            if not getattr(self, "stale_scale_ok", False) or age % WSCALE_EVERY == 0:
                mx = max(float(w.abs().max()) for w in ws)
                self.w_scale = 2.0 ** math.floor(math.log2(2048.0 / mx)) if mx > 0 else 1.0
            self._ws_age = age + 1
            cps = self.split_coutp()
            kts = pad32(self.Ktot)
            per = T * cps * kts
            if self.need_split:
                if self.whi is None:
                    self.whi = torch.empty(self.G * per, dtype=torch.float16, device=dev)
                    self.wlo = torch.empty(self.G * per, dtype=torch.float16, device=dev)
                for g, wd in enumerate(ws):
                    _lib.check(L.egne_pack_conv_weight_f16x2(wd.data_ptr(), self.Cout, self.Cin, self.kh, self.kw, cps, kts,
                                                             self.w_scale, self.whi.data_ptr() + 2 * g * per,
                                                             self.wlo.data_ptr() + 2 * g * per, st), "pack_f16x2")
            if self.need_sfrag:
                packs = self._sfrag_packs
                for cw in packs:
                    perf = T * cw * kts
                    if packs[cw] is None:
                        packs[cw] = (torch.empty(self.G * perf, dtype=torch.float16, device=dev),
                                     torch.empty(self.G * perf, dtype=torch.float16, device=dev))
                    for g, wd in enumerate(ws):
                        _lib.check(L.egne_pack_conv_weight_f16frag(wd.data_ptr(), self.Cout, self.Cin, self.kh, self.kw, cw, kts,
                                                                   self.w_scale, packs[cw][0].data_ptr() + 2 * g * perf,
                                                                   packs[cw][1].data_ptr() + 2 * g * perf, st), "pack_f16frag")
                self._sfrag_select()
        self._versions = vers
        return True

    def want_sfrag(self):
        self.need_sfrag = True
        self.__dict__.setdefault("_sfrag_packs", {}).setdefault(self.sfrag_coutp(), None)

    def _sfrag_ready(self):
        packs = getattr(self, "_sfrag_packs", {})
        return bool(packs) and all(v is not None for v in packs.values())

    def _sfrag_select(self):
        pk = self._sfrag_packs.get(self.sfrag_coutp())
        if pk is not None:
            self.fhi, self.flo = pk

    def sfrag_coutp(self):
        if self.CoutP == 96 and getattr(self, "halo_wide96", False):
            return 96
        return self.CoutP if self.CoutP <= 64 else (self.CoutP + 63) // 64 * 64

    def split_coutp(self):
        return (self.Cout + 127) // 128 * 128 if (self.Cout > 64 and self.G == 1) else self.CoutP

    def out_hw(self, H, W):
        d = self.dils[0]
        ho = (H + 2 * self.pad[0] * d - d * (self.kh - 1) - 1) // self.stride + 1
        wo = (W + 2 * self.pad[1] * d - d * (self.kw - 1) - 1) // self.stride + 1
        return ho, wo


def _pack_b1(layer, dev, st):
    L = _lib.lib()
    d = _lib.ConvDesc()
    d.nseg, d.CoutP, d.Ktot = len(layer.in_layout), layer.CoutP, layer.Ktot
    for i, (_, cp) in enumerate(layer.in_layout):
        d.seg[i].Cp = cp
    if getattr(layer, "b1frag", None) is None:
        n = int(L.egne_conv1x1_bf16_pack_elems(C.byref(d)))
        assert n > 0, "too many k-steps for the streaming 1x1 kernel"
        layer.b1frag = torch.empty(n, dtype=torch.bfloat16, device=dev)
        kofs, o = [], 0
        for _, cp in layer.in_layout:
            kofs.append(o)
            o += cp
        layer.b1info = torch.tensor(kofs + [cp for _, cp in layer.in_layout], dtype=torch.int32, device=dev)
    _lib.check(L.egne_pack_conv1x1_bf16(C.byref(d), layer.wp.data_ptr(), layer.b1info.data_ptr(), layer.b1frag.data_ptr(), st), "pack_conv1x1_bf16")


class PlanarPiece(Piece):

    def __init__(self, buf):
        assert buf.dim() == 4 and buf.shape[1] <= 4 and buf.is_contiguous()
        self.buf, self.off, self.C, self.Cp, self.n0 = buf, 0, int(buf.shape[1]), 8, 0
        self.scale = self.shift = None
        self.act_in = ACT_NONE
        self.nograd = True

    @property
    def stride(self):
        return 1

    @property
    def ptr(self):
        return self.buf.data_ptr()

    def with_norm(self, *a, **k):
        raise RuntimeError("a planar one-channel input cannot carry a fused normalisation")


class DgradLayer(ConvLayer):

    def __init__(self, fwd, idx, span=1):
        assert fwd.stride == 1 and fwd.pad_mode == 0 and fwd.G == 1, "dgrad: stride-1 zero-padded convs only"
        self.fwd, self.idx = fwd, idx
        self.ci0 = sum(c for c, _ in fwd.in_layout[:idx])
        assert span == 1 or all(c == cp for c, cp in fwd.in_layout[idx:idx + span])
        C_, Cp_ = sum(c for c, _ in fwd.in_layout[idx:idx + span]), sum(cp for _, cp in fwd.in_layout[idx:idx + span])
        self.weights, self.biases = fwd.weights, None
        self.in_layout = [(fwd.Cout, fwd.Cout_store)]
        self.Cout, self.Cin = C_, fwd.Cout
        self.kh, self.kw = fwd.kh, fwd.kw
        self.stride, self.pad_mode, self.act = 1, 0, ACT_NONE
        self.pad = (fwd.kh - 1 - fwd.pad[0], fwd.kw - 1 - fwd.pad[1])
        self.dils = fwd.dils
        self.Ktot, self.CoutP, self.Cout_store, self.G = fwd.Cout_store, pad32(C_), Cp_, 1
        self.wp = self.wf = self.bp = None
        self.need_flat = self.need_frag = False
        self.split = self.need_split = self.need_sfrag = False
        self.split1 = self.need_s1 = False
        self.s1hi = self.s1lo = None
        self.need_big, self.wimg = False, None
        self.need_big1, self.wimg1 = False, None
        self.need_m1, self.m1hi, self.m1lo = False, None, None
        self.need_c4h, self.c4hi, self.c4lo = False, None, None
# ... 438 lines not shown
        bw.raw(L.egne_act_norm_bwd, (g.ptr, g.stride, g.off, piece.ptr, piece.stride, piece.off, ACT_NONE, pend["scale"].data_ptr(), pend["shift"].data_ptr(),
                                     a1.ptr if a1 is not None else None, a1.stride if a1 is not None else 0, a1.off if a1 is not None else 0,
                                     gq.ptr if gq is not None else None, gq.stride if gq is not None else 0, gq.off if gq is not None else 0,
                                     pend["act_q"], piece.Cp, B, H, W, sums.data_ptr(), wsn.data_ptr(), None, 0, wsb.data_ptr(), B), name + ".norm_bwd_fused")

    def build_backward(self):
        bw = Plan(self.device, dtype=self.dtype)
        bw.fwd = self
        bw.dyn_scales = self.dyn_scales
        bw.serial_timing = True
        self._touching, self._touched = True, {}
        for emit in reversed(self.tape):
            emit(bw)
        self._touching = False
        assert not self._pending, "deferred normalisation gradients without a producer to take them: %s" % list(self._pending)
        self._zero_free = set()
        if ZERO_SKIP:
            for bid, ents in self._touched.items():
                cuts = sorted({e for ent in ents for e in ent[3:5]})
                ok = True
                for s0, s1 in zip(cuts, cuts[1:]):
                    cov = []
                    for a, b_, st, e0, e1 in ents:
                        if e1 <= s0 or e0 >= s1:
                            continue
                        if st:
                            cov.append((a, b_))
                            continue
                        need = [(a, b_)]
                        for ca, cb in cov:
                            need = [r for x0, x1 in need for r in ((x0, min(x1, ca)), (max(x0, cb), x1)) if r[0] < r[1]]
                        if need:
                            ok = False
                            break
                    if not ok:
                        break
                if ok:
                    self._zero_free.add(bid)
        self.bw = bw
        return bw

    def zero_grads(self):
        free = getattr(self, "_zero_free", ())
        ts = [t for bid, t in self.gtwins.items() if bid not in free]
        if not ts:
            return
        key = tuple(t.data_ptr() for t in ts)
        if self._ztable is None or self._ztable[0] != key:
            rows, blk = [], 0
            for t in ts:
                nb = t.numel() * t.element_size()
                assert t.is_contiguous() and t.data_ptr() % 16 == 0 and nb % 16 == 0
                rows.append((t.data_ptr(), nb, blk))
                blk += (nb + 65535) // 65536
            self._ztable = (key, torch.tensor(rows, dtype=torch.int64).to(self.device), blk)
        _, tab, blk = self._ztable
        _lib.check(self.L.egne_zero_many(tab.data_ptr(), len(ts), blk, _lib.stream_ptr()))

    def zero_grads_ahead(self):
        if not ZERO_AHEAD:
            return
        if self._zstream is None:
            self._zstream, self._zevent = torch.cuda.Stream(device=self.device), torch.cuda.Event()
            for t in self.gtwins.values():
                t.record_stream(self._zstream)
        self._zstream.wait_stream(torch.cuda.current_stream())
        with torch.cuda.stream(self._zstream):
            self.zero_grads()
        if self._ztable is not None:
            self._ztable[1].record_stream(self._zstream)
        self._zevent.record(self._zstream)
        self._zero_pending = True

    def zero_grads_join(self):
        if self._zero_pending:
            torch.cuda.current_stream().wait_event(self._zevent)
            self._zero_pending = False
        else:
            self.zero_grads()

    def ovf_ptr(self):
        if not OVF_CHECK or self.train or self.bf16 or self.dyn_scales or getattr(self, "fwd", None) is not None:
            return None
        if self.ovf is None:
            self.ovf = self.vec(1, dtype=torch.int32)
            self.ovf_host = torch.zeros(1, dtype=torch.int32).pin_memory()
            self.ovf_event = torch.cuda.Event()
        return self.ovf.data_ptr()

    OVF_MIRROR_EVERY = 16

    def _ovf_publish(self):
        if self.ovf is None:
            return
        self._ovf_runs = getattr(self, "_ovf_runs", 0) + 1
        if self._ovf_runs % self.OVF_MIRROR_EVERY or torch.cuda.is_current_stream_capturing():
            return
        self.ovf_host.copy_(self.ovf, non_blocking=True)
        self.ovf_event.record()
        self._ovf_recorded = True

    def _ovf_reset(self):
        self.ovf.zero_()
        self.ovf_host.zero_()
        self.calibrated = False
        self.overflow_events += 1

    def overflowed(self, wait=True):
        if self.ovf is None:
            return False
        if wait:
            if int(self.ovf.item()) == 0:
                return False
        else:
            if (not getattr(self, "_ovf_recorded", False) or torch.cuda.is_current_stream_capturing() or not self.ovf_event.query()
                    or int(self.ovf_host[0]) == 0):
                return False
        self._ovf_reset()
        return True

    def check_overflow(self):
        if not self.overflowed():
            return False
        self.run()
        if self.overflowed():
            raise RuntimeError("non-finite values in a split-f16 convolution after re-calibration: the inputs themselves are not finite")
        return True

    DYN_SLOTS = 512

    def _new_slot(self):
        if self.dynbuf is None:
            self.dynbuf = self.vec(self.DYN_SLOTS, dtype=torch.int32)
            self.pre.append(self.dynbuf.zero_)
        assert self.ndyn < self.DYN_SLOTS, "too many device-scaled launches in one plan"
        self.ndyn += 1
        return self.dynbuf.data_ptr() + 4 * (self.ndyn - 1)

    def _publish_absmax(self, piece, B):
        ptr = self._new_slot()
        self._absmax_of[(id(piece.buf), piece.off, piece.Cp, piece.n0, B)] = (ptr, len(self.calls))
        return ptr

    def _dyn_slot(self, d, pieces, B, npix, name):
        if self._dyn_hint is not None:
            d.dyn_scale = self._dyn_hint
            return
        if len(pieces) == 1:
            pc = pieces[0]
            ent = self._absmax_of.get((id(pc.buf), pc.off, pc.Cp, pc.n0, B))
            if ent is not None and len(self.calls) - ent[1] <= 4:
                d.dyn_scale = ent[0]
                return
        ptr = self._new_slot()
        for pc in pieces:
            self._add(self.L.egne_absmax, (pc.ptr, pc.stride, pc.off, pc.Cp, npix, ptr), name + ".absmax", kind="absmax")
        d.dyn_scale = ptr

    def _add(self, fn, args, name, flops=0.0, kind=None, cal=None, side=False, ws=()):
        for ai, layer, attr in ws:
            assert args[ai] == getattr(layer, attr), (name, ai, attr)
            self.wscale_refs.append((len(self.calls), ai, layer, attr))
        if cal is not None and CALIBRATE:
            self.cal[len(self.calls)] = cal
        if side or self.side_default:
            self.side_calls[len(self.calls)] = None
        if name == WINDOW_NAME and self.window_at is None and not self.train:
            self.window_at = len(self.calls)
        self.calls.append((fn, args, name))
        self.meta.append((kind or name.split(".")[0], flops))

    def _stats_ws(self, d, B, nchunk):
        ws = self.vec(B * nchunk * int(d.Cout_store) * 2, dtype=torch.float64)
        d.stats_ws, d.stats_nchunk = ws.data_ptr(), nchunk
        return ws

    def _stats_finish(self, ws, d, B, HW, nchunk, name, eps=1e-5):
        Cs = int(d.Cout_store)
        scale, shift = self.vec(B, Cs), self.vec(B, Cs)
        self._add(self.L.egne_norm_stats_finish, (ws.data_ptr(), Cs, B, nchunk, HW, eps, scale.data_ptr(), shift.data_ptr()),
                  name + ".stats", kind="norm_stats")
        return scale, shift

    def _conv_query(self, layer, pieces, dst, B, H, W, residual=None, stats=False, scores=None, pool=None, up_add=None):
        q = _lib.ConvQuery()
        q.dtype, q.B, q.H, q.W = (1 if self.bf16 else 0), B, H, W
        q.kh, q.kw, q.stride, q.pad_h, q.pad_w, q.pad_mode, q.ngroups = layer.kh, layer.kw, layer.stride, layer.pad[0], layer.pad[1], layer.pad_mode, layer.G
        for g in range(_lib.MAXGROUP):
            q.dil[g] = layer.dils[g] if g < layer.G else 1
        q.nseg = len(pieces)
        for i, p in enumerate(pieces):
            q.seg_C[i], q.seg_Cp[i], q.seg_ch_off[i], q.seg_pix_stride[i] = p.C, p.Cp, getattr(p, "off", 0), getattr(p, "stride", 0)
            q.seg_affine[i] = int(p.scale is not None)
        p0 = pieces[0]
        q.seg_planar, q.seg_presplit = int(isinstance(p0, PlanarPiece)), int(getattr(p0, "presplit", None) is not None)
        if getattr(p0, "split3", None) is not None:
            q.seg_presplit = 3
        q.Cout, q.Cout_store = layer.Cout, layer.Cout_store
        if dst is not None:
            q.dst_Cp, q.dst_ch_off, q.dst_pix_stride = dst.Cp, dst.off, dst.stride
        q.act, q.has_post, q.has_residual = layer.act, int(layer.post is not None), int(residual is not None)
        if residual is not None:
            q.res_pix_stride, q.res_ch_off = residual.stride, residual.off
        q.split, q.split1, q.split_c4 = int(bool(layer.split)), int(bool(layer.split1)), int(bool(getattr(layer, "split_c4", False)))
        q.train, q.dyn_scales = int(bool(self.train)), int(bool(self.dyn_scales))
        q.is_dgrad = int(isinstance(layer, (DgradLayer, SplitDgradLayer, BfDgradLayer)))
        q.want_stats, q.want_scores = int(bool(stats)), int(scores is not None)
        if pool is not None:
            q.want_pool, q.pool_Cp, q.pool_pix_stride = 1, pool.Cp, pool.stride
        q.up_add = int(bool(up_add))
        q.f16_products = int(self.f16_products)
        q.f16_storage = int(getattr(p0, "f16s", None) is not None or (dst is not None and dst.f16s is not None))
        return q

    def msdil_ok(self, layer, piece, H, W):
        return choose_conv(self._conv_query(layer, [piece], piece, 1, H, W, residual=piece), self.L).kind == "conv_f16x3:msdil"

    def stream1x1_ok(self, layer, pieces, B, H, W, up_add=False):
        return len(pieces) <= _lib.MAXSEG and choose_conv(self._conv_query(layer, pieces, None, B, H, W, up_add=up_add), self.L).kind == "conv_f16x3:stream1x1"

    def bf16_stream1x1_ok(self, layer, pieces, dst, B, H, W):
        return len(pieces) <= _lib.MAXSEG and choose_conv(self._conv_query(layer, pieces, dst, B, H, W), self.L).kind == "conv_bf16:1x1"

    def _check_dispatch(self, q, choice, name):
        ch = _lib.ConvChoice()
        _lib.check(self.L.egne_conv2d_auto_kind(C.byref(q), C.byref(ch)), "conv2d_auto_kind")
        mine = (choice.kind, bool(choice.tail_frames), choice.fused_pool, choice.fused_stats)
        theirs = (ch.name.decode(), bool(ch.tail_frames), bool(ch.fused_pool), bool(ch.fused_stats))
        DISPATCH_LOG.append((name, mine[0], theirs[0]))
        assert mine == theirs, "%s: the planner chose %s (kind, frame tail, pooled output, statistics), egne_conv2d_auto_kind %s" % (name, mine, theirs)

    def conv(self, layer, pieces, dst, B, H, W, residual=None, name="conv", stats=False, scores=None, pool=None, up_add=None, partials=False):
        self.last_pooled = self.last_presplit = False
        r = self._conv_impl(layer, pieces, dst, B, H, W, residual, name, stats, scores, pool, up_add, partials)
        def esz_of(p):
            if getattr(p, "f16s", None) is not None:
                return 2.0
            if self.f16_products == 1 and getattr(p, "presplit", None) is not None:
                return 2.0
            return float(self.esz)
        LAYER_BYTES[name] = B * (H * W * sum(p.Cp * esz_of(p) for p in pieces) + r[0] * r[1] * (min(layer.Cout_store, dst.Cp) * esz_of(dst) + (residual.Cp * esz_of(residual) if residual is not None else 0)))
        return r

    def _apply_choice(self, layer, choice, p0):
        needs, _, sfrag, _ = _KIND[choice.kind]
        for flag in needs + (("need_big1",) if choice.big1 else ()) + (("need_split",) if choice.tail_frames else ()):
            setattr(layer, flag, True)
        if choice.kind == "conv_bf16:3x3" and self.train:
            layer.need_flat = True
        if choice.kind == "conv_f16x3:msdil" and p0.presplit is not None:
            layer.k_perm = SPLIT_PAIR_PERM
        layer.halo_wide96 = choice.halo_wide96
        if sfrag:
            layer.want_sfrag()
        if layer not in self.layers:
            self.layers.append(layer)
        layer.ensure_packed(self.device)

    def _desc(self, layer, pieces, dst, B, H, W, Ho, Wo, residual=None, dtype=0):
        d = _lib.ConvDesc()
        d.dtype = dtype
        d.ovf_flag, d.f16_products = self.ovf_ptr(), self.f16_products
        d.B, d.H, d.W, d.Ho, d.Wo = B, H, W, Ho, Wo
        d.kh, d.kw, d.stride = layer.kh, layer.kw, layer.stride
        d.pad_h, d.pad_w, d.pad_mode = layer.pad[0], layer.pad[1], layer.pad_mode
        d.ngroups = layer.G
        for g in range(_lib.MAXGROUP):
            d.dil[g] = layer.dils[g] if g < layer.G else 1
        d.nseg = len(pieces)
        for i, p in enumerate(pieces):
            s = d.seg[i]
            s.ptr, s.pix_stride, s.ch_off, s.Cp = p.ptr, p.stride, p.off, p.Cp
            s.scale = p.scale.data_ptr() if p.scale is not None else None
            s.shift = p.shift.data_ptr() if p.shift is not None else None
            s.act_in = p.act_in
        d.bias = layer.bp.data_ptr() if layer.biases is not None else None
        d.act = layer.act
        if layer.post is not None:
            d.post_scale, d.post_shift = layer.post[0].data_ptr(), layer.post[1].data_ptr()
        if residual is not None:
            d.residual, d.res_pix_stride, d.res_ch_off = residual.ptr, residual.stride, residual.off
        if dst is not None:
            d.out, d.out_pix_stride, d.out_ch_off = dst.ptr, dst.stride, dst.off
            d.Cout_store = min(layer.Cout_store, dst.Cp)
            assert tuple(dst.buf.shape[1:3]) == (Ho, Wo), (tuple(dst.buf.shape), Ho, Wo)
        self.keep.append(d)
        return d

    def _storage_rules(self, cv):
        choice, kind, layer, dst, p0, d = cv.choice, cv.choice.kind, cv.layer, cv.dst, cv.pieces[0], cv.d
        big, rsrw = kind == "conv_f16x3:big", kind in ("conv_f16x3:rw", "conv_f16x3:rs")
        calibrated = CALIBRATE and not self.dyn_scales and cv.raw
        fin, fout = getattr(p0, "f16s", None), dst.f16s
        if fin is not None or fout is not None:
            if not (rsrw or kind == "conv_f16x3:first" or (big and choice.big1)) or (big and not calibrated):
                raise NeedsFp32Storage(cv.name)
            if rsrw and (not (kind == "conv_f16x3:rw" and self.f16_products == 1 and calibrated and layer.post is None and cv.residual is None)
                         or (fout is None and choice.fused_pool)):
                raise NeedsFp32Storage(cv.name)
        in3, out3 = getattr(p0, "split3", None), dst.split3
        if in3 is not None or out3 is not None:
            halo3 = (kind == "conv_f16x3:halo" and out3 is None and layer.dils[0] == 1
                     and layer.sfrag_coutp() == 32 and not cv.stats and cv.pool is None)
            if not ((big or halo3) and not (big and choice.big1) and self.f16_products != 1 and calibrated and not self.train
                    and p0.Cp % 32 == 0 and p0.off % 32 == 0 and (out3 is None or (int(d.Cout_store) % 32 == 0 and dst.off % 32 == 0))):
                raise NeedsFp32Storage(cv.name)

    def _calibration(self, cv):
        B, H, W = cv.B, cv.H, cv.W
        cv.cal3 = (3, list(cv.pieces), B * H * W) if cv.raw else None
        cv.cal2 = (2, list(cv.pieces), B * H * W) if cv.raw else None
        if self.dyn_scales:
            cv.layer.stale_scale_ok = True
        if self.dyn_scales and cv.raw and _KIND[cv.choice.kind][1]:
            self._dyn_slot(cv.d, cv.pieces, B, B * H * W, cv.name)
            cv.cal3 = cv.cal2 = None
        in3 = getattr(cv.pieces[0], "split3", None)
        if in3 is not None:
            cv.d.seg[0].presplit = 3
            cv.cal2 = (lambda args, vmax, in3=in3: args[:2] + (in3.value,) + args[3:], [], 0)
            cv.cal3 = (lambda args, vmax, in3=in3: args[:3] + (in3.value,) + args[4:], [], 0)

    def _conv_impl(self, layer, pieces, dst, B, H, W, residual, name, stats, scores, pool, up_add, partials):
        assert len(pieces) == len(layer.in_layout) and len(pieces) <= _lib.MAXSEG, name
        for p, (c, cp) in zip(pieces, layer.in_layout):
            assert p.Cp == cp and p.C == c, (name, p.C, p.Cp, c, cp)
        q = self._conv_query(layer, pieces, dst, B, H, W, residual, stats, scores, pool, up_add)
        if self.bf16:
            return self._conv_bf16(q, layer, pieces, dst, B, H, W, residual, name, stats, scores, up_add, partials)
        choice = choose_conv(q, self.L)
        kind, p0 = choice.kind, pieces[0]
        planar = isinstance(p0, PlanarPiece)
        assert not planar or kind == "conv_f16x3:first", "%s: only the first-layer streaming kernel reads planar inputs" % name
        assert planar or p0.presplit is None or kind == "conv_f16x3:msdil", "%s: only the one-launch dilated group reads split-pair storage" % name
        assert scores is None or kind == "conv_f16x3:msdil", "score fusion needs the one-launch MSBlock kernel (check Plan.msdil_ok first)"
        assert up_add is None or kind == "conv_f16x3:stream1x1", "%s: an up-sampled addend needs the streaming 1x1 kernel (check Plan.stream1x1_ok first)" % name
        self._apply_choice(layer, choice, p0)
        Ho, Wo = layer.out_hw(H, W)
        d = self._desc(layer, pieces, dst, B, H, W, Ho, Wo, residual)
        if planar:
            d.seg[0].Cp = p0.C
        _, split, sfrag, _ = _KIND[kind]
        big = kind == "conv_f16x3:big"
        d.Ktot = pad32(layer.Ktot) if split else layer.Ktot
        d.CoutP = layer.big_coutp if big else layer.sfrag_coutp() if sfrag else layer.split_coutp() if split else layer.CoutP
        d.w = (layer.wimg if big else layer.fhi if sfrag else layer.whi if split else layer.wf if kind == "conv3x3_halo" else layer.wp).data_ptr()
        cv = types.SimpleNamespace(choice=choice, layer=layer, pieces=pieces, dst=dst, d=d, B=B, H=H, W=W, Ho=Ho, Wo=Wo, residual=residual, name=name,
                                   stats=stats, scores=scores, pool=pool, up_add=up_add, raw=all(pc.scale is None for pc in pieces),
                                   flops=2.0 * B * Ho * Wo * layer.Cout * layer.Cin * layer.kh * layer.kw * layer.G)
        self._storage_rules(cv)
        self._calibration(cv)
        took_stats = getattr(self, _KIND[kind][3])(cv)
        if CHECK_DISPATCH:
            self._check_dispatch(q, choice, name)
        if stats and not took_stats:
            self.last_stats = self.norm_stats(dst, B, Ho * Wo, name=name + ".stats")[:2]
        if self.train:
            db = _lib.ConvDesc()
            C.memmove(C.byref(db), C.byref(d), C.sizeof(_lib.ConvDesc))
            db.B, db.Ktot, db.CoutP = B, layer.Ktot, layer.CoutP
            db.seg[0].ptr, db.out = pieces[0].ptr, dst.ptr
            self.keep.append(db)
            self.tape.append(lambda bw: self._bw_conv(bw, layer, list(pieces), dst, db, B, H, W, Ho, Wo, name))
        return Ho, Wo

    def _emit_narrow_f32(self, cv):
        layer, d, p0 = cv.layer, cv.d, cv.pieces[0]
        cp32 = (p0.Cp + 31) // 32 * 32
        wn = self.vec(9 * cp32 * 4)

        def repack(layer=layer, wn=wn):
            w = layer.weights[0].detach().to(torch.float32).contiguous()
            _lib.check(self.L.egne_pack_conv3x3_narrow_weight(w.data_ptr(), layer.Cout, layer.Cin, wn.data_ptr(), _lib.stream_ptr()), "pack_conv3x3_narrow")
        self.pre.append(VersionGuard([layer.weights[0]], repack))
        d.Ktot, d.CoutP, d.w = cp32, 4, wn.data_ptr()
        assert int(self.L.egne_conv3x3_narrow_supported(C.byref(d))) == 1 and p0.act_in == ACT_NONE, cv.name
        self._add(self.L.egne_conv3x3_narrow_fwd, (C.byref(d),), cv.name, flops=2.0 * cv.B * cv.H * cv.W * layer.Cout * layer.Cin * 9, kind="conv3x3_narrow")

    def _emit_big(self, cv):
        layer, d, dst, p0, choice, B = cv.layer, cv.d, cv.dst, cv.pieces[0], cv.choice, cv.B
        npix, tail, cal2 = B * cv.Ho * cv.Wo, choice.tail_frames, cv.cal2
        if dst.f16s is not None:
            cal2 = self._f16_out(d, layer, dst, npix, cal2, p0.f16s)
        if getattr(p0, "f16s", None) is not None:
            cal2 = self._f16_in(d, p0.f16s, cal2, 2)
        launches = [(len(self.calls), d)]
        if tail:
            d2 = _lib.ConvDesc()
            C.memmove(C.byref(d2), C.byref(d), C.sizeof(_lib.ConvDesc))
            d.B, d2.B = B - tail, tail
            d2.seg[0].ptr = p0.ptr + 4 * (B - tail) * cv.H * cv.W * p0.stride
            d2.out = dst.ptr + 4 * (B - tail) * cv.Ho * cv.Wo * dst.stride
            d2.Ktot, d2.CoutP = pad32(layer.Ktot), layer.split_coutp()
            self.keep.append(d2)
            launches.append((len(self.calls) + 1, d2))
        self._add(self.L.egne_conv2d_f16_big1_fwd if choice.big1 else self.L.egne_conv2d_f16x3_big_fwd,
                  (C.byref(d), (layer.wimg1 if choice.big1 else layer.wimg).data_ptr(), F16X3_ASCALE, layer.w_scale_big), cv.name,
                  flops=cv.flops * (B - tail) / B if tail else cv.flops, kind="conv_f16x3:big", cal=cal2, ws=[(3, layer, "w_scale_big")])
        if tail:
            self._add(self.L.egne_conv2d_f16x3_fwd, (C.byref(d2), layer.whi.data_ptr(), layer.wlo.data_ptr(), F16X3_ASCALE, layer.w_scale),
                      cv.name + ".tail", flops=cv.flops * tail / B, kind="conv_f16x3:flat", cal=cv.cal3, ws=[(4, layer, "w_scale")])
        if dst.split3 is not None:
            self._split3_out(launches, dst, npix)

    def _emit_gemm1x1(self, cv):
        layer, d = cv.layer, cv.d
        d.Ktot, d.CoutP = layer.m1_ktot, layer.m1_coutp
        self._add(self.L.egne_conv1x1_ms_f16x3_fwd, (C.byref(d), layer.m1hi.data_ptr(), layer.m1lo.data_ptr(), F16X3_ASCALE,
                                                     layer.w_scale_m1), cv.name, flops=cv.flops, kind="conv_f16x3:gemm1x1", cal=cv.cal3, ws=[(4, layer, "w_scale_m1")])

    def _emit_stream1x1(self, cv):
        layer, d = cv.layer, cv.d
        if cv.up_add is not None:
            P, ph, pw = cv.up_add
            assert (2 * ph, 2 * pw) == (cv.H, cv.W) and layer.act == ACT_NONE and P.Cp >= int(d.Cout_store) and tuple(P.buf.shape[:3]) == (cv.B, ph, pw), cv.name
            d.Ho, d.Wo = ph, pw
            d.residual, d.res_pix_stride, d.res_ch_off = P.ptr, P.stride, P.off
        self._add(self.L.egne_conv1x1_f16x3_fwd, (C.byref(d), layer.s1hi.data_ptr(), layer.s1lo.data_ptr(), F16X3_ASCALE,
                                                  layer.w_scale1), cv.name, flops=cv.flops, kind="conv_f16x3:stream1x1", cal=cv.cal3, ws=[(4, layer, "w_scale1")])

    def _emit_msdil(self, cv):
        layer, d = cv.layer, cv.d
        cal3 = self._presplit_in(d, cv.pieces, cv.residual, cv.cal3)
        fn, heads = self.L.egne_msblock_dil_f16_fwd, ()
        if cv.scores is not None:
            cw_, cc_, s0_, s1_, accum = cv.scores
            fn, heads, d.out = self.L.egne_msblock_dil_scores_f16_fwd, (cw_.data_ptr(), cc_.data_ptr(), s0_.data_ptr(), s1_.data_ptr(), int(accum)), None
        self._add(fn, (C.byref(d), layer.fhi.data_ptr(), layer.flo.data_ptr(), F16X3_ASCALE, layer.w_scale) + heads, cv.name, flops=cv.flops,
                  kind="conv_f16x3:msdil", cal=cal3, ws=[(4, layer, "w_scale")])

    def _emit_lattice(self, cv):
        layer, d, dst = cv.layer, cv.d, cv.dst
        perf = 9 * layer.sfrag_coutp() * pad32(layer.Ktot)
        for g in range(3):
            dg = _lib.ConvDesc()
            C.memmove(C.byref(dg), C.byref(d), C.sizeof(_lib.ConvDesc))
            dg.ngroups = 1
            dg.dil[0] = layer.dils[g]
            dg.bias = layer.bp.data_ptr() + 4 * g * layer.CoutP if layer.biases is not None else None
            if g > 0:
                dg.residual, dg.res_pix_stride, dg.res_ch_off = dst.ptr, dst.stride, dst.off
            self.keep.append(dg)
            self._add(self.L.egne_conv3x3_halo_f16_fwd, (C.byref(dg), layer.fhi.data_ptr() + 2 * g * perf,
                                                         layer.flo.data_ptr() + 2 * g * perf, F16X3_ASCALE, layer.w_scale),
                      cv.name + ".g%d" % g, flops=cv.flops / 3, kind="conv_f16x3:lattice", cal=cv.cal3, ws=[(4, layer, "w_scale")])

    def _emit_rs_rw(self, cv):
        layer, d, dst, pieces, choice, pq = cv.layer, cv.d, cv.dst, cv.pieces, cv.choice, cv.pool
        B, H, W, name, cal3 = cv.B, cv.H, cv.W, cv.name, cv.cal3
        rw = choice.kind == "conv_f16x3:rw"
        if choice.fused_pool:
            d.pool_out, d.pool_pix_stride, d.pool_ch_off = pq.ptr, pq.stride, pq.off
            self.last_pooled = True
        th = 8 if pieces[0].Cp <= 32 else 4
        nchunk = ((W + 31) // 32) * ((H + th - 1) // th) * (2 if (th == 4 and layer.sfrag_coutp() >= 64) else 4)
        if choice.fused_stats:
            ws = self._stats_ws(d, B, nchunk)
        ps = dst.presplit
        if (ps is not None and rw and cv.raw and CALIBRATE and not self.dyn_scales and layer.post is None and cv.residual is None
                and not self.last_pooled and int(d.Cout_store) % 32 == 0 and dst.off % 32 == 0):
            d.out_split, d.out_split_scale = 1, ps.value
            self.last_presplit = True

            def cal_ps(args, vmax, d=d, layer=layer, ps=ps):
                with torch.no_grad():
                    bound = vmax * float(layer.weights[0].detach().abs().sum(dim=(1, 2, 3)).max())
                    if layer.biases is not None and layer.biases[0] is not None:
                        bound += float(layer.biases[0].detach().abs().max())
                ps.value = d.out_split_scale = _a_scale_for(bound)
                return args[:3] + (_a_scale_for(vmax),) + args[4:]
            cal3 = (cal_ps, list(pieces), B * H * W)
        fin, fout = pieces[0].f16s, dst.f16s
        if fout is not None:
            assert not choice.fused_pool or pq.f16s is fout, "%s: the pooled second output shares the main output's storage scale" % name
            cal3 = self._f16_out(d, layer, dst, B * cv.Ho * cv.Wo, cal3, fin)
        if fin is not None:
            cal3 = self._f16_in(d, fin, cal3, 3)
        self._add(self.L.egne_conv3x3_rw_f16_fwd if rw else self.L.egne_conv3x3_rs_f16_fwd,
                  (C.byref(d), layer.fhi.data_ptr(), layer.flo.data_ptr(), F16X3_ASCALE, layer.w_scale), name, flops=cv.flops,
                  kind=choice.kind, cal=cal3, ws=[(4, layer, "w_scale")])
        if choice.fused_stats:
            self.last_stats = self._stats_finish(ws, d, B, H * W, nchunk, name)
        return choice.fused_stats

    def _emit_halo(self, cv):
        layer, d, choice, pq, H, W = cv.layer, cv.d, cv.choice, cv.pool, cv.H, cv.W
        tx, ty = (W + 31) // 32, (H + 7) // 8
        if ((H + 31) // 32) * ((W + 7) // 8) < tx * ty and HALO_TALL:
            tx, ty = (H + 31) // 32, (W + 7) // 8
        if choice.fused_pool:
            d.pool_out, d.pool_pix_stride, d.pool_ch_off = pq.ptr, pq.stride, pq.off
            self.last_pooled = True
        if choice.fused_stats:
            ws = self._stats_ws(d, cv.B, tx * ty * 4)
        self._add(self.L.egne_conv3x3_halo_f16_fwd, (C.byref(d), layer.fhi.data_ptr(), layer.flo.data_ptr(), F16X3_ASCALE,
                                                     layer.w_scale), cv.name, flops=cv.flops, kind="conv_f16x3:halo", cal=cv.cal3, ws=[(4, layer, "w_scale")])
        if choice.fused_stats:
            self.last_stats = self._stats_finish(ws, d, cv.B, H * W, tx * ty * 4, cv.name)
        return choice.fused_stats

    def _emit_small(self, cv):
        layer, small_ws = cv.layer, cv.choice.small_ws
        wsb = self.vec(max(small_ws, 4))
        self._add(self.L.egne_conv2d_f16x3_small_fwd, (C.byref(cv.d), layer.whi.data_ptr(), layer.wlo.data_ptr(), F16X3_ASCALE,
                                                       layer.w_scale, wsb.data_ptr(), small_ws), cv.name, flops=cv.flops,
                  kind="conv_f16x3:small", cal=cv.cal3, ws=[(4, layer, "w_scale")])

    def _emit_flat(self, cv):
        self._add(self.L.egne_conv2d_f16x3_fwd, (C.byref(cv.d), cv.layer.whi.data_ptr(), cv.layer.wlo.data_ptr(), F16X3_ASCALE,
                                                 cv.layer.w_scale), cv.name, flops=cv.flops, kind="conv_f16x3:flat", cal=cv.cal3, ws=[(4, cv.layer, "w_scale")])

    def _emit_first(self, cv):
        layer, d, cal3 = cv.layer, cv.d, cv.cal3
        d.CoutP = layer.c4_coutp
        if cv.dst.f16s is not None:
            cal3 = self._f16_out(d, layer, cv.dst, cv.B * cv.Ho * cv.Wo, cal3, None)
        self._add(self.L.egne_conv3x3_smallcin_f16_fwd, (C.byref(d), layer.c4hi.data_ptr(), layer.c4lo.data_ptr(), F16X3_ASCALE,
                                                         layer.w_scale_c4), cv.name, flops=cv.flops, kind="conv_f16x3:first", cal=cal3, ws=[(4, layer, "w_scale_c4")])

    def _emit_smallcin(self, cv):
        self._add(self.L.egne_conv3x3_smallcin_fwd, (C.byref(cv.d), cv.layer.w40.data_ptr()), cv.name, flops=cv.flops, kind="conv3x3_smallcin")

    def _emit_halo_f32(self, cv):
        self._add(self.L.egne_conv3x3_halo_fwd, (C.byref(cv.d),), cv.name, flops=cv.flops, kind="conv3x3_halo")

    def _emit_igemm(self, cv):
        if self.dyn_scales and cv.residual is None and int(cv.d.Cout_store) >= cv.dst.Cp:
            cv.d.absmax_out = self._publish_absmax(cv.dst, cv.B)
        self._add(self.L.egne_conv2d_fwd, (C.byref(cv.d),), cv.name, flops=cv.flops, kind="conv_igemm")

    def _emit_bf16_3x3(self, cv):
        self._add(self.L.egne_conv3x3_bf16_fwd, (C.byref(cv.d), cv.layer.bfrag.data_ptr()), cv.name, flops=cv.flops, kind="conv_bf16:3x3")
        self._last_b3_desc = cv.d

    def _emit_bf16_1x1(self, cv):
        self._add(self.L.egne_conv1x1_bf16_fwd, (C.byref(cv.d), cv.layer.b1frag.data_ptr()), cv.name, flops=cv.flops, kind="conv_bf16:1x1")

    def _emit_bf16_narrow(self, cv):
        self._add(self.L.egne_conv_narrow_bf16_fwd, (C.byref(cv.d),), cv.name, flops=cv.flops, kind="conv_bf16:narrow")

    def _conv_bf16(self, q, layer, pieces, dst, B, H, W, residual, name, stats, scores, up_add, partials):
        assert scores is None and layer.G == 1 and not isinstance(pieces[0], PlanarPiece), name
        assert dst.buf.dtype == torch.bfloat16 and all(p.buf.dtype == torch.bfloat16 for p in pieces), name
        choice = choose_conv(q, self.L)
        self._apply_choice(layer, choice, pieces[0])
        Ho, Wo = layer.out_hw(H, W)
        d = self._desc(layer, pieces, dst, B, H, W, Ho, Wo, residual, dtype=1)
        wp = getattr(layer, "wp", None)
        d.Ktot, d.CoutP, d.w = layer.Ktot, layer.CoutP, (wp.data_ptr() if wp is not None else None)
        if choice.kind == "conv_igemm" and BF16_NARROW:
            q.narrow_bf16_ok = int(self.L.egne_conv_narrow_bf16_supported(C.byref(d)))
            choice = choose_conv(q, self.L)
        kind = choice.kind
        if kind == "conv_bf16:3x3":
            d.Ktot, d.w = pad32(layer.Ktot), None
        assert up_add is None or (kind == "conv_bf16:1x1" and residual is None and layer.act == ACT_NONE), "%s: an up-sampled addend needs the streaming bf16 1x1 kernel" % name
        db = None
        if self.train:
            db = _lib.ConvDesc()
            C.memmove(C.byref(db), C.byref(d), C.sizeof(_lib.ConvDesc))
            db.Ktot, db.CoutP = layer.Ktot, layer.CoutP
            self.keep.append(db)
        ws_stats, self.last_partials = None, None
        if (stats or partials) and kind == "conv_bf16:3x3" and STATS_FUSED and STATS_FUSED_BF16 and self.train:
            nchunk_s = ((W + 31) // 32) * ((H + 7) // 8) * 4
            ws_stats = self._stats_ws(d, B, nchunk_s)
            if partials:
                self.last_partials = (ws_stats, nchunk_s, int(d.Cout_store))
        if up_add is not None:
            P, ph, pw = up_add
            assert (2 * ph, 2 * pw) == (H, W) and P.Cp >= int(d.Cout_store) and tuple(P.buf.shape[:3]) == (B, ph, pw) and P.off % 8 == 0 and P.stride % 8 == 0, name
            d.Ho, d.Wo = ph, pw
            d.residual, d.res_pix_stride, d.res_ch_off = P.ptr, P.stride, P.off
        cv = types.SimpleNamespace(choice=choice, layer=layer, d=d, dst=dst, B=B, residual=residual, name=name,
                                   flops=2.0 * B * Ho * Wo * layer.Cout * layer.Cin * layer.kh * layer.kw)
        getattr(self, _KIND[kind][3])(cv)
        if CHECK_DISPATCH:
            self._check_dispatch(q, choice, name)
        if stats:
            self.last_stats = (self._stats_finish(ws_stats, d, B, Ho * Wo, nchunk_s, name) if ws_stats is not None
                               else self.norm_stats(dst, B, Ho * Wo, name=name + ".stats")[:2])
        if self.train:
            def emit(bw, up_add=up_add):
                self._bw_conv(bw, layer, list(pieces), dst, db, B, H, W, Ho, Wo, name)
                if up_add is not None:
                    P, ph, pw = up_add
                    Pq = Piece(P.buf, P.off, min(P.C, int(db.Cout_store)), int(db.Cout_store), P.n0)
                    first = self.first_touch(Pq.buf, Pq.off, Pq.Cp, Pq.n0, B)
                    gz, gP = self.gp(dst, B), self.gp(Pq, B)
                    if first:
                        self.mark_stored(Pq, B)
                    bw.raw(self.L.egne_upsample2x_bwd_store if first else self.L.egne_upsample2x_bwd,
                           (gz.ptr, gz.stride, gz.off, gP.ptr, gP.stride, gP.off, B, ph, pw, Pq.Cp), name + ".up_add.bwd")
            self.tape.append(emit)
        return Ho, Wo

    def _f16_out(self, d, layer, dst, npix, cal, fin):
        fs = dst.f16s
        assert self.f16_products == 1 and CALIBRATE and not self.dyn_scales and cal is not None, "f16 storage needs a calibrated plain-f16 plan"
        d.out_split, d.out_split_scale = 2, fs.value
        ai, pcs, npx = cal

        def cal_out(args, vmax, d=d, layer=layer, fs=fs, ai=ai, fin=fin):
            if fin is not None and not vmax:
                vmax = getattr(fin, "vmax", None) or 2047.0 / fin.value
            with torch.no_grad():
                bound = vmax * float(layer.weights[0].detach().abs().sum(dim=(1, 2, 3)).max())
                if layer.biases is not None and layer.biases[0] is not None:
                    bound += float(layer.biases[0].detach().abs().max())
            fs.value = d.out_split_scale = _a_scale_for(bound)
            return ai(args, vmax) if callable(ai) else args[:ai] + (_a_scale_for(vmax),) + args[ai + 1:]
        self.post_cal[len(self.calls)] = (d, dst, fs, npix)
        return (cal_out, pcs, npx)

    def _split3_out(self, launches, dst, npix):
        ss = dst.split3
        for _, dd in launches:
            dd.out_split, dd.out_split_scale = 3, ss.value
        self.post_cal3[launches[-1][0]] = (launches, dst, ss, npix)

    def _f16_in(self, d, fin, cal, ai):
        d.seg[0].presplit = 2
        inner = cal[0] if (cal is not None and callable(cal[0])) else None

        def cal_in(args, vmax, fin=fin, inner=inner, ai=ai):
            if inner is not None:
                args = inner(args, getattr(fin, "vmax", None) or 2047.0 / fin.value)
            return args[:ai] + (fin.value,) + args[ai + 1:]
        return (cal_in, [], 0)

    def _presplit_in(self, d, pieces, residual, cal):
        ps = pieces[0].presplit
        if ps is None:
            return cal
        assert residual is not None and residual.buf is pieces[0].buf and residual.off == pieces[0].off, "split-pair input must be the residual too"
        d.seg[0].presplit = 1
        return (lambda args, vmax, ps=ps: args[:3] + (ps.value,) + args[4:], [], 0)

    def pair_fusable(self, l1, pieces, l2, dst, H, W):
        return (FUSE_1X1 and F16X3_ENABLED and not self.train and not self.bf16 and l1.split1 and l2.split and l1.kh == 1 and l1.kw == 1
                and l1.stride == 1 and l1.G == 1 and l1.pad == (0, 0) and l1.act == ACT_NONE and l1.post is None
                and all(pc.scale is None for pc in pieces) and l1.CoutP in (32, 64) and len(pieces) <= _lib.MAXSEG
                and sum((pc.Cp + 15) // 16 for pc in pieces) <= 12
                and l2.kh == 3 and l2.kw == 3 and l2.stride == 1 and l2.G == 1 and l2.pad == (1, 1) and l2.dils[0] == 1
                and l2.pad_mode == 0 and len(l2.in_layout) == 1 and l2.in_layout[0][0] == l1.Cout and l2.CoutP in (32, 64)
                and W >= FUSE_1X1_MIN_W and all(H * W * pc.stride < 2 ** 29 for pc in pieces) and H * W * dst.stride < 2 ** 29)

    def td_pool_fusable(self, layer, pieces, dst):
        G = sum((p.Cp + 15) // 16 for p in pieces)
        return (TDPOOL_FUSED and F16X3_ENABLED and not self.train and not self.bf16 and layer.split1 and layer.kh == 1 and layer.kw == 1 and layer.stride == 1
                and layer.G == 1 and layer.post is None and all(p.scale is not None for p in pieces) and len(pieces) <= _lib.MAXSEG
                and layer.CoutP <= 96 and G * (layer.CoutP // 32) * 2048 <= 80 * 1024 and dst.Cp % 4 == 0)

    def conv1x1_pooled(self, layer, pieces, dst, B, H, W, name="td", stats=False):
        assert self.td_pool_fusable(layer, pieces, dst), name
        Ho, Wo = H // 2, W // 2
        layer.need_s1 = layer.need_flat = True
        if layer not in self.layers:
            self.layers.append(layer)
        layer.ensure_packed(self.device)
        assert tuple(layer.pad) == (0, 0) and layer.pad_mode == 0, name
        d = self._desc(layer, pieces, dst, B, H, W, Ho, Wo)
        d.dil[0:_lib.MAXGROUP] = (0,) * _lib.MAXGROUP
        d.Ktot, d.CoutP = layer.Ktot, layer.CoutP
        flops = 2.0 * B * Ho * Wo * layer.Cout * layer.Cin
        TN = layer.CoutP // 32
        lds = sum((p.Cp + 15) // 16 for p in pieces) * TN * 2048 + 4 * 32 * 36 * 4
        fuse_stats = stats and STATS_FUSED and dst.Cp == int(d.Cout_store) and lds <= 80 * 1024
        if fuse_stats:
            bpf = (Ho * Wo + 31) // 32
            cb = max(1, min(8, B * bpf // TDPOOL_STATS_UNITS))
            nchunk = (bpf + cb - 1) // cb
            ws = self._stats_ws(d, B, nchunk)
        self._add(self.L.egne_conv1x1_pool2_f16x3_fwd, (C.byref(d), layer.s1hi.data_ptr(), layer.s1lo.data_ptr(), F16X3_ASCALE, layer.w_scale1),
                  name, flops=flops, kind="conv_f16x3:tdpool1x1", ws=[(4, layer, "w_scale1")])
        LAYER_BYTES[name] = 4.0 * B * (H * W * sum(p.Cp for p in pieces) + Ho * Wo * int(d.Cout_store))
        if fuse_stats:
            self.last_stats = self._stats_finish(ws, d, B, Ho * Wo, nchunk, name)
        elif stats:
            self.last_stats = self.norm_stats(dst, B, Ho * Wo, name=name + ".stats")[:2]
        return Ho, Wo

    def conv_pair(self, l1, pieces, l2, dst, B, H, W, tmp=None, residual=None, name="pair", stats=False, up_add=None):
        r = self._conv_pair_impl(l1, pieces, l2, dst, B, H, W, tmp, residual, name, stats, up_add)
        LAYER_BYTES[name] = 4.0 * B * H * W * (sum(p.Cp for p in pieces) + min(l2.Cout_store, dst.Cp) + (residual.Cp if residual is not None else 0)
                                               + (8 if up_add is not None else 0))
        return r

    def _conv_pair_impl(self, l1, pieces, l2, dst, B, H, W, tmp=None, residual=None, name="pair", stats=False, up_add=None):
        fused = self.pair_fusable(l1, pieces, l2, dst, H, W)
        assert up_add is None or self.bf16 or (fused and l1.CoutP == 32 and l2.CoutP == 32 and sum((pc.Cp + 15) // 16 for pc in pieces) <= 8), name
        fused_c4 = (FUSE_1X1 and FUSE_C4 and F16X3_ENABLED and not self.train and not self.bf16 and l1.split and l2.split and l1.kh == 3 and l1.kw == 3
                    and l1.stride == 1 and l1.G == 1 and l1.pad == (1, 1) and l1.pad_mode == 0 and l1.dils[0] == 1 and l1.Cin <= 4
                    and l1.post is None and len(pieces) == 1 and pieces[0].scale is None and pieces[0].Cp >= 4 and l1.CoutP == 32
                    and l2.kh == 3 and l2.kw == 3 and l2.stride == 1 and l2.G == 1 and l2.pad == (1, 1) and l2.dils[0] == 1
                    and l2.pad_mode == 0 and len(l2.in_layout) == 1 and l2.in_layout[0][0] == l1.Cout and l2.CoutP == 32
                    and W >= FUSE_1X1_MIN_W and H * W * pieces[0].stride < 2 ** 29 and H * W * dst.stride < 2 ** 29
                    and (not isinstance(pieces[0], PlanarPiece) or l1.Cin == 1))
        assert fused_c4 or not isinstance(pieces[0], PlanarPiece), "%s: only the fused convBlock kernel reads planar inputs" % name
        if fused_c4:
            return self._conv_pair_c4(l1, pieces[0], l2, dst, B, H, W, residual, name, stats)
        if not fused:
            if tmp is None:
                tmp = Piece(self.buf(B, H, W, pad8(l1.Cout)), 0, l1.Cout)
            if (PAIR_BIAS and self.train and l1.act == ACT_NONE and l1.biases is not None and l2.biases is not None and l1.G == 1
                    and l2.G == 1 and l2.kh == 3 and l2.kw == 3 and l2.pad == (1, 1) and l2.dils[0] == 1 and l2.stride == 1
                    and l2.pad_mode == 0 and l1.Cout <= 256 and pad8(l2.Cout) <= 256 and l2.Cin == l1.Cout):
                self._pair_links[id(l1)] = l2
                self._pair_links[id(l2)] = l1
            self.conv(l1, pieces, tmp, B, H, W, name=name + ".a", up_add=up_add)
            return self.conv(l2, [tmp], dst, B, H, W, residual=residual, name=name + ".b", stats=stats)
        for p, (c, cp) in zip(pieces, l1.in_layout):
            assert p.Cp == cp and p.C == c, (name, p.C, p.Cp, c, cp)
        l1.need_s1 = True
        l1.need_flat = True
        l2.want_sfrag()
        for l in (l1, l2):
            if l not in self.layers:
                self.layers.append(l)
            l.ensure_packed(self.device)
        d1 = self._desc(l1, pieces, None, B, H, W, H, W)
        d1.ovf_flag, d1.f16_products = None, 0
        d1.Ktot, d1.CoutP = l1.Ktot, l1.CoutP
        if up_add is not None:
            P, ph, pw = up_add
            assert (2 * ph, 2 * pw) == (H, W) and P.Cp >= 32 and tuple(P.buf.shape[:3]) == (B, ph, pw)
            d1.Ho, d1.Wo = ph, pw
            d1.residual, d1.res_pix_stride, d1.res_ch_off = P.ptr, P.stride, P.off
        d2 = self._desc(l2, [], dst, B, H, W, H, W, residual)
        d2.Ktot, d2.CoutP = l1.CoutP, l2.sfrag_coutp()

        def rescale(args, vmax, l1=l1, up_add=up_add):
            with torch.no_grad():
                w = l1.weights[0].detach()
                bound = vmax * float(w.abs().sum(dim=(1, 2, 3)).max())
                if l1.biases is not None and l1.biases[0] is not None:
                    bound += float(l1.biases[0].detach().abs().max())
                if up_add is not None:
                    bound += float(up_add[0].buf[..., up_add[0].off:up_add[0].off + up_add[0].Cp].abs().max())
            return args[:4] + (_a_scale_for(vmax),) + args[5:8] + (_a_scale_for(bound),) + args[9:]
        flops = 2.0 * B * H * W * (l1.Cout * l1.Cin + l2.Cout * l2.Cin * 9)
        fuse_stats = stats and STATS_FUSED and dst.Cp == int(d2.Cout_store)
        if fuse_stats:
            th = 8 if l1.CoutP == 32 else 4
            nchunk = ((W + 31) // 32) * ((H + th - 1) // th) * (2 if (l1.CoutP == 64 and d2.CoutP == 64) else 4)
            ws = self._stats_ws(d2, B, nchunk)
        self._add(self.L.egne_conv1x1_3x3_fused_f16_fwd,
                  (C.byref(d1), C.byref(d2), l1.s1hi.data_ptr(), l1.s1lo.data_ptr(), F16X3_ASCALE, l1.w_scale1,
                   l2.fhi.data_ptr(), l2.flo.data_ptr(), F16X3_ASCALE, l2.w_scale), name, flops=flops, kind="conv_f16x3:fused1x1",
                  cal=(rescale, list(pieces), B * H * W), ws=[(5, l1, "w_scale1"), (9, l2, "w_scale")])
        if fuse_stats:
            self.last_stats = self._stats_finish(ws, d2, B, H * W, nchunk, name)
        elif stats:
            self.last_stats = self.norm_stats(dst, B, H * W, name=name + ".stats")[:2]
        return H, W

    def _conv_pair_c4(self, l1, src, l2, dst, B, H, W, residual, name, stats):
        l1.need_c4h = True
        l1.need_flat = True
        l2.want_sfrag()
        for l in (l1, l2):
            if l not in self.layers:
                self.layers.append(l)
            l.ensure_packed(self.device)
        assert l1.c4_coutp == 32
        d1 = self._desc(l1, [src], None, B, H, W, H, W)
        d1.ovf_flag, d1.f16_products = None, 0
        d1.Ktot, d1.CoutP = src.Cp, 32
        d2 = self._desc(l2, [], dst, B, H, W, H, W, residual)
        d2.Ktot, d2.CoutP = 32, 32
        if C1V and isinstance(src, PlanarPiece) and l1.Cin == 1 and l1.Cout <= 32:
            w12 = self.vec(32, 12)

            def refresh_w12(w12=w12, l1=l1):
                with torch.no_grad():
                    w12.zero_()
                    w12[:l1.Cout, :9].copy_(l1.weights[0].detach().reshape(l1.Cout, 9))
                    if l1.biases is not None and l1.biases[0] is not None:
                        w12[:l1.Cout, 9].copy_(l1.biases[0].detach())
            self.pre.append(VersionGuard([l1.weights[0]] + ([l1.biases[0]] if l1.biases is not None and l1.biases[0] is not None else []), refresh_w12))
            d1.w = w12.data_ptr()

        def rescale(args, vmax, l1=l1):
            with torch.no_grad():
                bound = vmax * float(l1.weights[0].detach().abs().sum(dim=(1, 2, 3)).max())
                if l1.biases is not None and l1.biases[0] is not None:
                    bound += float(l1.biases[0].detach().abs().max())
            return args[:4] + (_a_scale_for(vmax),) + args[5:8] + (_a_scale_for(bound),) + args[9:]
        flops = 2.0 * B * H * W * 9 * (l1.Cout * l1.Cin + l2.Cout * l2.Cin)
        fuse_stats = stats and STATS_FUSED and dst.Cp == int(d2.Cout_store)
        nchunk = ((W + 31) // 32) * ((H + 7) // 8) * 4
        if fuse_stats:
            ws = self._stats_ws(d2, B, nchunk)
        self._add(self.L.egne_conv3x3c4_3x3_fused_f16_fwd,
                  (C.byref(d1), C.byref(d2), l1.c4hi.data_ptr(), l1.c4lo.data_ptr(), F16X3_ASCALE, l1.w_scale_c4,
                   l2.fhi.data_ptr(), l2.flo.data_ptr(), F16X3_ASCALE, l2.w_scale), name, flops=flops, kind="conv_f16x3:fused3x3c4",
                  cal=(rescale, [src], B * H * W), ws=[(5, l1, "w_scale_c4"), (9, l2, "w_scale")])
        if fuse_stats:
            self.last_stats = self._stats_finish(ws, d2, B, H * W, nchunk, name)
        elif stats:
            self.last_stats = self.norm_stats(dst, B, H * W, name=name + ".stats")[:2]
        return H, W

    def _bw_conv(self, bw, layer, pieces, dst, d, B, H, W, Ho, Wo, name):
        L = self.L
        Cs = int(d.Cout_store)
        npix = B * Ho * Wo
        masked = None
        pend = self._pending.pop((id(dst.buf), dst.off, dst.n0), None) if self._pending else None
        cand = self._mask_cands.get((id(dst.buf), dst.off, Cs, dst.n0, B, Ho, Wo)) if (MASK_ON_WRITE and self.bf16 and pend is None) else None
        if cand is not None:
            ents = self._touched.get(id(dst.buf), [])
            last = max((i for i, e in enumerate(ents) if e[0] < dst.off + dst.Cp and e[1] > dst.off), default=-1)
            needs_sums = (layer.biases is not None and layer.biases[0] is not None) or id(layer) in self._pair_links
            taken = any(q.sums for q in cand[1])
            if last == cand[0] and layer.act in (ACT_NONE, ACT_RELU, ACT_LEAKY) and (not needs_sums or (not taken and pad32(Cs) <= 128)):
                masked = cand
        masked3 = None
        cand3 = self._mask_cands3.get((id(dst.buf), dst.off, Cs, dst.n0, B, Ho, Wo)) if (MASK3_ON_WRITE and self.bf16 and pend is None and masked is None) else None
# ... 524 lines not shown
```

Baseline: 2217.

## Store stem conv outputs as presplit f16 hi/lo pairs for conv1_2 and pool

```diff
diff --git a/edge-guided-near-eye-image-analysis-for-head-mounted-displays_amd/bdcn_new.py b/edge-guided-near-eye-image-analysis-for-head-mounted-displays_amd/bdcn_new.py
--- a/edge-guided-near-eye-image-analysis-for-head-mounted-displays_amd/bdcn_new.py
+++ b/edge-guided-near-eye-image-analysis-for-head-mounted-displays_amd/bdcn_new.py
@@ -109,12 +109,17 @@
                 else:
                     p.normal_(0, 0.01)
 
-    def _build(self, B, H, W, dev, only_fuse, edge_thres, f16_storage=None, split3=False):
+    def _build(self, B, H, W, dev, only_fuse, edge_thres, f16_storage=None, split3=False, stem=0):
         if f16_storage is None:
             h8, w8 = (maxpool_out(maxpool_out(maxpool_out(n, 2), 2), 2) for n in (H, W))
-            if engine.PRESPLIT_TRUNK and engine.CALIBRATE and getattr(self, "_plan_products", 0) != 1 and B * h8 * w8 >= 256 * 128:
+            three = engine.CALIBRATE and getattr(self, "_plan_products", 0) != 1
+            trunk = bool(engine.PRESPLIT_TRUNK and three and B * h8 * w8 >= 256 * 128)
+            stem_on = min(int(engine.PRESPLIT_STEM), 1) if (three and B * H * W >= engine.PRESPLIT_STEM_MIN_PIX) else 0
+            for t, s in dict.fromkeys(((True, stem_on), (True, 0), (False, stem_on))):
+                if (t and not trunk) or not (t or s):
+                    continue
                 try:
-                    return self._build(B, H, W, dev, only_fuse, edge_thres, 0, True)
+                    return self._build(B, H, W, dev, only_fuse, edge_thres, 0, t, s)
                 except engine.NeedsFp32Storage:
                     pass
             if engine.F16_STORAGE and getattr(self, "_plan_products", 0) == 1:
@@ -127,6 +132,7 @@
         pl = Plan(dev)
         pl.f16_storage = int(f16_storage)
         pl.split3_trunk = bool(split3)
+        pl.split3_stem = int(stem)
         pl.f16_products = getattr(self, "_plan_products", 0)
         L = pl.L
         f = self.features
@@ -263,13 +269,14 @@
             dst = Piece(ob, 0, cout)
             if h16:
                 dst.f16s = engine.SplitScale()
-            if split3 and name[4] in "345":
+            if (split3 and name[4] in "345") or (stem >= 1 and name in ("conv1_1", "conv1_2")):
                 dst.split3 = engine.SplitScale()
             nxt = _VGG[idx + 1] if idx + 1 < len(_VGG) else None
             pq = None
             if nxt is not None and nxt[0] == "P" and nxt[1] == 2:
                 pq = Piece((pl.buf16 if h16 else pl.buf)(B, maxpool_out(hh, 2), maxpool_out(ww, 2), pad8(cout)), 0, cout)
                 pq.f16s = dst.f16s
+                pq.split3 = dst.split3
             pl.conv(layer, [cur], dst, B, hh, ww, name="vgg." + name, pool=pq)
             pooled = pq if pl.last_pooled else None
             cur = dst
diff --git a/edge-guided-near-eye-image-analysis-for-head-mounted-displays_amd/csrc/conv3x3_c4_f16.hip b/edge-guided-near-eye-image-analysis-for-head-mounted-displays_amd/csrc/conv3x3_c4_f16.hip
--- a/edge-guided-near-eye-image-analysis-for-head-mounted-displays_amd/csrc/conv3x3_c4_f16.hip
+++ b/edge-guided-near-eye-image-analysis-for-head-mounted-displays_amd/csrc/conv3x3_c4_f16.hip
@@ -119,6 +119,14 @@
           if (tn == 0 && j == 0) bad |= egne_nonfinite((float)h0[0]);
           const u32x2 two = {__builtin_bit_cast(unsigned, h0), __builtin_bit_cast(unsigned, h1)};
           __builtin_amdgcn_raw_buffer_store_b64(two, ro, n < p.Cout_store ? (li * (int)p.out_pix_stride + p.out_ch_off + n) * 2 : (int)OOB, 0, 0);
+        } else if (p.out_split == 3) {
+          h2 h0, h1, l0, l1;
+          egne::split2(v[0], v[1], p.out_split_scale, h0, l0);
+          egne::split2(v[2], v[3], p.out_split_scale, h1, l1);
+          const u32x2 hi = {__builtin_bit_cast(unsigned, h0), __builtin_bit_cast(unsigned, h1)}, lo = {__builtin_bit_cast(unsigned, l0), __builtin_bit_cast(unsigned, l1)};
+          const int off = n < p.Cout_store ? (li * (int)p.out_pix_stride + p.out_ch_off + tn * 32) * 4 + (8 * j + 4 * kq) * 2 : (int)OOB;
+          __builtin_amdgcn_raw_buffer_store_b64(hi, ro, off, 0, 0);
+          __builtin_amdgcn_raw_buffer_store_b64(lo, ro, off, 64, 0);
         } else
         __builtin_amdgcn_raw_buffer_store_b128(__builtin_bit_cast(u32x4, v), ro,
                                                n < p.Cout_store ? (li * (int)p.out_pix_stride + p.out_ch_off + n) * 4 : (int)OOB, 0, 0);
@@ -170,7 +178,8 @@
                d.out_pix_stride * 128 < (1ll << 31) && (!d.bias || ((uintptr_t)d.bias & 15) == 0) &&
                (!d.post_scale || (((uintptr_t)d.post_scale & 15) == 0 && ((uintptr_t)d.post_shift & 15) == 0)), "conv_smallcin_f16: output");
   EGNE_REQUIRE(((uintptr_t)fhi & 15) == 0 && ((uintptr_t)flo & 15) == 0 && a_scale > 0.f && w_scale > 0.f, "conv_smallcin_f16: weights / scales");
-  EGNE_REQUIRE(d.out_split == 0 || (d.out_split == 2 && d.out_split_scale > 0.f && !d.post_scale), "conv_smallcin_f16: f16 output (out_split = 2) needs a positive scale and no post affine");
+  EGNE_REQUIRE(d.out_split == 0 || ((d.out_split == 2 || d.out_split == 3) && d.out_split_scale > 0.f && !d.post_scale), "conv_smallcin_f16: f16 / split-pair output (out_split = 2, 3) needs a positive scale and no post affine");
+  EGNE_REQUIRE(d.out_split != 3 || (d.f16_products != 1 && d.Cout_store % 32 == 0 && d.out_ch_off % 32 == 0), "conv_smallcin_f16: split-pair output (out_split = 3) needs three products and whole 32-channel blocks");
   const long long M = (long long)d.B * d.H * d.W;
   const long long nb = (M + 31) / 32;
   EGNE_REQUIRE(nb < (1ll << 31), "conv_smallcin_f16: too many pixels");
diff --git a/edge-guided-near-eye-image-analysis-for-head-mounted-displays_amd/csrc/conv3x3_rw_f16.hip b/edge-guided-near-eye-image-analysis-for-head-mounted-displays_amd/csrc/conv3x3_rw_f16.hip
--- a/edge-guided-near-eye-image-analysis-for-head-mounted-displays_amd/csrc/conv3x3_rw_f16.hip
+++ b/edge-guided-near-eye-image-analysis-for-head-mounted-displays_amd/csrc/conv3x3_rw_f16.hip
@@ -13,10 +13,11 @@
 constexpr int WCH = 9 * 2 * 2 * 512;
 constexpr int NI = (NPX * 8 + 255) / 256;
 
-template <int KCH, int NP = 3, bool F16IN = false, int SH = 0>
+template <int KCH, int NP = 3, int INF = 0, int SH = 0>
 __global__ __launch_bounds__(512)
 void conv3x3_rw_kernel(const egne_conv_desc p, const _Float16* __restrict__ fhi, const _Float16* __restrict__ flo, float a_scale,
                        float out_scale, int tiles_x, int tiles_y, int ntiles, int ncb, int nrun) {
+  constexpr bool F16IN = INF == 2, IN3 = INF == 3;
   egne::dyn_scales(p.dyn_scale, a_scale, out_scale);
   extern __shared__ __attribute__((aligned(16))) _Float16 ldsh[];
   _Float16* const lw = ldsh + 2 * IMGH;
@@ -70,7 +71,9 @@
     constexpr int NPC = F16IN ? 4 : 8, PGS = 256 / NPC, CPP = 32 / NPC, ESZ = F16IN ? 2 : 4, NQ = (NPX * NPC + 255) / 256;
     const int piece = tid & (NPC - 1), pg = tid / NPC;
     const float slope_in = sg.act_in == EGNE_ACT_RELU ? 0.f : (sg.act_in == EGNE_ACT_LEAKY ? 0.01f : 1.f);
-    const int lofs = F16IN ? pg * 32 + ((piece ^ ((pg >> 1) & 3)) << 3) : pg * 32 + (((piece >> 1) ^ ((pg >> 1) & 3)) << 3) + ((piece & 1) << 2);
+    const int lofs = F16IN ? pg * 32 + ((piece ^ ((pg >> 1) & 3)) << 3)
+                   : IN3 ? (piece >> 2) * (NPX * 32) + pg * 32 + (((piece & 3) ^ ((pg >> 1) & 3)) << 3)
+                         : pg * 32 + (((piece >> 1) ^ ((pg >> 1) & 3)) << 3) + ((piece & 1) << 2);
     u32x4 st[2][NQ];
     int rel[NQ];
 #pragma unroll
@@ -114,7 +117,7 @@
     auto convert1 = [&](const Job& jb, _Float16* img, auto bc, auto ic) {
       constexpr int BUF = decltype(bc)::value, I = decltype(ic)::value;
       const int px = pg + PGS * I;
-      if constexpr (F16IN) {
+      if constexpr (F16IN || IN3) {
         if (I < NQ - 1 || px < NPX) *(u32x4*)&img[lofs + 32 * PGS * I] = st[BUF][I];
         return;
       }
@@ -219,7 +222,8 @@
     const int l15 = lane & 15, kg = lane >> 4;
     const bool o16 = GEN && NP == 1 && p.out_split == 2;
     const bool split_on = SH == 4 || (GEN && !o16 && p.out_split != 0);
-    const bool pool_on = SH == 3 || (GEN && p.pool_out != nullptr);
+    constexpr bool OUT3 = SH == 6 || SH == 7;
+    const bool pool_on = SH == 3 || SH == 7 || (GEN && p.pool_out != nullptr);
     const bool full_epi = SH == 5 || (GEN && (p.post_scale != nullptr || p.residual != nullptr));
     const int oesz = o16 ? 2 : 4;
     const unsigned frame_out = (unsigned)H * W * (unsigned)p.out_pix_stride * (unsigned)oesz;
@@ -254,6 +258,10 @@
       lco[ph] = (xl[ph] * (int)p.out_pix_stride + p.out_ch_off + cb * 32 + 4 * kg) * oesz;
       lcr[ph] = (xl[ph] * (int)p.res_pix_stride + p.res_ch_off + cb * 32 + 4 * kg) * 4;
       lcp[ph] = ((xl[ph] >> 1) * (int)p.pool_pix_stride + p.pool_ch_off + cb * 32 + 4 * kg) * oesz;
+      if constexpr (OUT3) {
+        lco[ph] = (xl[ph] * (int)p.out_pix_stride + p.out_ch_off + cb * 32) * 4 + 8 * kg;
+        lcp[ph] = ((xl[ph] >> 1) * (int)p.pool_pix_stride + p.pool_ch_off + cb * 32) * 4 + 8 * kg;
+      }
     }
     f32x4 R[2][2][2][2];
 #pragma unroll
@@ -280,7 +288,14 @@
             const float t = m * out_scale + b4[nh][e];
             v[e] = fmaxf(t, t * slope_out);
           }
-          if (o16) {
+          if constexpr (OUT3) {
+            h2 h0, h1, l0, l1;
+            egne::split2(v[0], v[1], p.out_split_scale, h0, l0);
+            egne::split2(v[2], v[3], p.out_split_scale, h1, l1);
+            const u32x2 hi = {__builtin_bit_cast(unsigned, h0), __builtin_bit_cast(unsigned, h1)}, lo = {__builtin_bit_cast(unsigned, l0), __builtin_bit_cast(unsigned, l1)};
+            __builtin_amdgcn_raw_buffer_store_b64(hi, rpo, jok[nh] ? poff : (int)OOB, nh * 32, 0);
+            __builtin_amdgcn_raw_buffer_store_b64(lo, rpo, jok[nh] ? poff : (int)OOB, 64 + nh * 32, 0);
+          } else if (o16) {
             const egne::sp_f32x2 u0 = {v[0] * p.out_split_scale, v[1] * p.out_split_scale}, u1 = {v[2] * p.out_split_scale, v[3] * p.out_split_scale};
             const h2 h0 = __builtin_convertvector(u0, h2), h1 = __builtin_convertvector(u1, h2);
             const u32x2 two = {__builtin_bit_cast(unsigned, h0), __builtin_bit_cast(unsigned, h1)};
@@ -315,7 +330,14 @@
         }
       }
       if constexpr (nh == 0) ovf_m = max(ovf_m, __builtin_bit_cast(unsigned, v[0]) & 0x7fffffffu);
-      if (o16) {
+      if constexpr (OUT3) {
+        h2 h0, h1, l0, l1;
+        egne::split2(v[0], v[1], p.out_split_scale, h0, l0);
+        egne::split2(v[2], v[3], p.out_split_scale, h1, l1);
+        const u32x2 hi = {__builtin_bit_cast(unsigned, h0), __builtin_bit_cast(unsigned, h1)}, lo = {__builtin_bit_cast(unsigned, l0), __builtin_bit_cast(unsigned, l1)};
+        __builtin_amdgcn_raw_buffer_store_b64(hi, rout, jok[nh] ? tvo : (int)OOB, nh * 32, 0);
+        __builtin_amdgcn_raw_buffer_store_b64(lo, rout, jok[nh] ? tvo : (int)OOB, 64 + nh * 32, 0);
+      } else if (o16) {
         const egne::sp_f32x2 u0 = {v[0] * p.out_split_scale, v[1] * p.out_split_scale}, u1 = {v[2] * p.out_split_scale, v[3] * p.out_split_scale};
         const h2 h0 = __builtin_convertvector(u0, h2), h1 = __builtin_convertvector(u1, h2);
         if constexpr (nh == 0) ovf_h = max(ovf_h, __builtin_bit_cast(unsigned, h0) & 0x7fffu);
@@ -384,13 +406,14 @@
                 c = __builtin_amdgcn_mfma_f32_16x16x32_f16(wh[Bq][nh], ah[Bq][tm][ph], c, 0, 0, 0);
                 R[P][tm][ph][nh] = c;
               }
-          constexpr int NM = NP == 3 ? 24 : 8, ND = t + 1 < 9 ? (NP == 3 ? 12 : 6) : 0, NV = FIRST && SH == 3 && t < 4 ? 4 : 3;
+          constexpr int NM = NP == 3 ? 24 : 8, ND = t + 1 < 9 ? (NP == 3 ? 12 : 6) : 0, NV = FIRST && (SH == 3 || SH == 7) && t < 4 ? 4 : 3;
+          constexpr int NS = SH == 7 && t < 4 ? 4 : 3;
           [&]<int... Ms>(std::integer_sequence<int, Ms...>) {
             (([&] {
               __builtin_amdgcn_sched_group_barrier(0x8, 1, 0);
               if constexpr (Ms < ND) __builtin_amdgcn_sched_group_barrier(0x100, 1, 0);
               __builtin_amdgcn_sched_group_barrier(0x2, NV, 0);
-              if constexpr (FIRST && Ms >= NM - 3) __builtin_amdgcn_sched_group_barrier(0x40, 1, 0);
+              if constexpr (FIRST && Ms >= NM - NS) __builtin_amdgcn_sched_group_barrier(0x40, 1, 0);
             }()), ...);
           }(std::make_integer_sequence<int, NM>{});
         }()), ...);
@@ -655,32 +678,44 @@
   }
 }
 
-template <int KCH, int NP, bool F16IN, int SH>
+template <int KCH, int NP, int INF, int SH>
 int launch_rw_form(const egne_conv_desc& d, const _Float16* fhi, const _Float16* flo, float a_scale, float os, hipStream_t st);
 
-template <int KCH, int NP = 3, bool F16IN = false>
+template <int KCH, int NP = 3, int INF = 0>
 int launch_rw(const egne_conv_desc& d, const _Float16* fhi, const _Float16* flo, float a_scale, float os, hipStream_t st) {
   const char* e = getenv("EGNE_RW_SHADOW");
-  if (e && e[0] == '0') return launch_rw_form<KCH, NP, F16IN, 0>(d, fhi, flo, a_scale, os, st);
-  if constexpr (NP == 3) {
-    if ((d.post_scale || d.residual) && d.pool_out) return launch_rw_form<KCH, NP, F16IN, 0>(d, fhi, flo, a_scale, os, st);
-    if (d.post_scale || d.residual) return launch_rw_form<KCH, NP, F16IN, 5>(d, fhi, flo, a_scale, os, st);
-    if (d.pool_out) return launch_rw_form<KCH, NP, F16IN, 3>(d, fhi, flo, a_scale, os, st);
-    if (d.out_split) return launch_rw_form<KCH, NP, F16IN, 4>(d, fhi, flo, a_scale, os, st);
-    return launch_rw_form<KCH, NP, F16IN, 2>(d, fhi, flo, a_scale, os, st);
+  if constexpr (INF == 3) {
+    if ((e && e[0] == '0') || d.post_scale || d.residual)
+      return egne::fail(EGNE_ERR_ARG, "conv3x3_rw: a split-pair input (presplit = 3) has the shadow form only, without post affine / residual");
+    if constexpr (KCH == 2) {
+      if (d.out_split == 3) return d.pool_out ? launch_rw_form<KCH, NP, INF, 7>(d, fhi, flo, a_scale, os, st) : launch_rw_form<KCH, NP, INF, 6>(d, fhi, flo, a_scale, os, st);
+      if (d.pool_out) return launch_rw_form<KCH, NP, INF, 3>(d, fhi, flo, a_scale, os, st);
+    } else {
+      if (d.out_split == 3 || d.pool_out) return egne::fail(EGNE_ERR_ARG, "conv3x3_rw: split-pair (3) / pooled output over a split-pair input needs a 64-channel slice");
+    }
+    if (d.out_split) return launch_rw_form<KCH, NP, INF, 4>(d, fhi, flo, a_scale, os, st);
+    return launch_rw_form<KCH, NP, INF, 2>(d, fhi, flo, a_scale, os, st);
+  } else if constexpr (NP == 3) {
+    if (e && e[0] == '0') return launch_rw_form<KCH, NP, INF, 0>(d, fhi, flo, a_scale, os, st);
+    if ((d.post_scale || d.residual) && d.pool_out) return launch_rw_form<KCH, NP, INF, 0>(d, fhi, flo, a_scale, os, st);
+    if (d.post_scale || d.residual) return launch_rw_form<KCH, NP, INF, 5>(d, fhi, flo, a_scale, os, st);
+    if (d.pool_out) return launch_rw_form<KCH, NP, INF, 3>(d, fhi, flo, a_scale, os, st);
+    if (d.out_split) return launch_rw_form<KCH, NP, INF, 4>(d, fhi, flo, a_scale, os, st);
+    return launch_rw_form<KCH, NP, INF, 2>(d, fhi, flo, a_scale, os, st);
   } else {
-    return launch_rw_form<KCH, NP, F16IN, 1>(d, fhi, flo, a_scale, os, st);
+    if (e && e[0] == '0') return launch_rw_form<KCH, NP, INF, 0>(d, fhi, flo, a_scale, os, st);
+    return launch_rw_form<KCH, NP, INF, 1>(d, fhi, flo, a_scale, os, st);
   }
 }
 
-template <int KCH, int NP, bool F16IN, int SH>
+template <int KCH, int NP, int INF, int SH>
 int launch_rw_form(const egne_conv_desc& d, const _Float16* fhi, const _Float16* flo, float a_scale, float os, hipStream_t st) {
   const int tiles_x = (d.W + TW - 1) / TW, tiles_y = (d.H + TH - 1) / TH;
   const int ntiles = tiles_x * tiles_y * d.B, ncb = d.CoutP / 32, nrun = (d.Cout_store + 31) / 32;
   constexpr size_t lds = ((size_t)2 * IMGH + (size_t)(KCH == 0 ? 2 : KCH) * WCH) * sizeof(_Float16);
   static_assert(lds <= 163840, "LDS budget");
-  if (!egne::raise_lds((const void*)conv3x3_rw_kernel<KCH, NP, F16IN, SH>, lds)) return egne::fail(EGNE_ERR_LAUNCH, "conv3x3_rw: cannot raise the dynamic LDS limit to %zu", lds);
-  hipLaunchKernelGGL((conv3x3_rw_kernel<KCH, NP, F16IN, SH>), dim3(256), dim3(512), lds, st, d, fhi, flo, a_scale, os, tiles_x, tiles_y, ntiles, ncb, nrun);
+  if (!egne::raise_lds((const void*)conv3x3_rw_kernel<KCH, NP, INF, SH>, lds)) return egne::fail(EGNE_ERR_LAUNCH, "conv3x3_rw: cannot raise the dynamic LDS limit to %zu", lds);
+  hipLaunchKernelGGL((conv3x3_rw_kernel<KCH, NP, INF, SH>), dim3(256), dim3(512), lds, st, d, fhi, flo, a_scale, os, tiles_x, tiles_y, ntiles, ncb, nrun);
   return egne::check_launch("egne_conv3x3_rw_f16_fwd");
 }
 
@@ -706,27 +741,36 @@
   EGNE_REQUIRE(((uintptr_t)fhi & 15) == 0 && ((uintptr_t)flo & 15) == 0 && a_scale > 0.f && w_scale > 0.f, "conv3x3_rw: weights / scales");
   EGNE_REQUIRE(d.out_split != 1 || (d.out_split_scale > 0.f && d.Cout_store % 32 == 0 && d.out_ch_off % 32 == 0 && !d.pool_out && !d.post_scale && !d.residual),
                "conv3x3_rw: split-pair output needs whole 32-channel blocks, a positive scale and no pooled / post-affine / residual options");
-  EGNE_REQUIRE(d.out_split == 0 || d.out_split == 1 || (d.out_split == 2 && d.f16_products == 1 && d.out_split_scale > 0.f && !d.post_scale && !d.residual),
+  EGNE_REQUIRE(d.out_split == 0 || d.out_split == 1 || d.out_split == 3 || (d.out_split == 2 && d.f16_products == 1 && d.out_split_scale > 0.f && !d.post_scale && !d.residual),
                "conv3x3_rw: f16 output (out_split = 2) needs f16_products = 1, a positive scale and no post-affine / residual options");
-  const bool in16 = g.presplit == 2;
-  EGNE_REQUIRE(g.presplit == 0 || (in16 && d.f16_products == 1 && !g.scale && g.ch_off % 8 == 0 && g.pix_stride % 8 == 0 &&
-                                   (long long)d.H * d.W * g.pix_stride * 2 < (1ll << 31)),
+  const bool in16 = g.presplit == 2, in3 = g.presplit == 3;
+  EGNE_REQUIRE(d.out_split != 3 || (in3 && d.out_split_scale > 0.f && d.Cout_store % 32 == 0 && d.out_ch_off % 32 == 0 && !d.post_scale && !d.residual &&
+                                    (!d.pool_out || d.pool_ch_off % 32 == 0)),
+               "conv3x3_rw: channel-order split-pair output (out_split = 3) needs a split-pair input, whole 32-channel blocks, a positive scale and no post-affine / residual options");
+  EGNE_REQUIRE(g.presplit == 0 || in3 || (in16 && d.f16_products == 1 && !g.scale && g.ch_off % 8 == 0 && g.pix_stride % 8 == 0 &&
+                                          (long long)d.H * d.W * g.pix_stride * 2 < (1ll << 31)),
                "conv3x3_rw: an f16 input slice (presplit = 2) needs f16_products = 1, no fused affine and 16-byte aligned pixels");
+  EGNE_REQUIRE(!in3 || (d.f16_products != 1 && !d.dyn_scale && !g.scale && g.Cp % 32 == 0 && g.ch_off % 32 == 0 && d.Ktot >= 64),
+               "conv3x3_rw: a split-pair input slice (presplit = 3) needs three products, a host-side scale, no fused affine and whole 32-channel blocks (two or more)");
   EGNE_REQUIRE((long long)d.H * d.W * g.pix_stride * 4 < (1ll << 31) && (long long)d.H * d.W * d.out_pix_stride * 4 < (1ll << 31) &&
                (!d.residual || (long long)d.H * d.W * d.res_pix_stride * 4 < (1ll << 31)), "conv3x3_rw: frame too large for 32-bit byte offsets");
   const float os = 1.0f / (a_scale * w_scale);
   hipStream_t st = (hipStream_t)stream;
   const _Float16 *h = (const _Float16*)fhi, *l = (const _Float16*)flo;
   if (d.f16_products == 1 && in16) {
-    if (d.Ktot == 32) return launch_rw<1, 1, true>(d, h, l, a_scale, os, st);
-    if (d.Ktot == 64) return launch_rw<2, 1, true>(d, h, l, a_scale, os, st);
-    return launch_rw<0, 1, true>(d, h, l, a_scale, os, st);
+    if (d.Ktot == 32) return launch_rw<1, 1, 2>(d, h, l, a_scale, os, st);
+    if (d.Ktot == 64) return launch_rw<2, 1, 2>(d, h, l, a_scale, os, st);
+    return launch_rw<0, 1, 2>(d, h, l, a_scale, os, st);
   }
   if (d.f16_products == 1) {
     if (d.Ktot == 32) return launch_rw<1, 1>(d, h, l, a_scale, os, st);
     if (d.Ktot == 64) return launch_rw<2, 1>(d, h, l, a_scale, os, st);
     return launch_rw<0, 1>(d, h, l, a_scale, os, st);
   }
+  if (in3) {
+    if (d.Ktot == 64) return launch_rw<2, 3, 3>(d, h, l, a_scale, os, st);
+    return launch_rw<0, 3, 3>(d, h, l, a_scale, os, st);
+  }
   if (d.Ktot == 32) return launch_rw<1>(d, h, l, a_scale, os, st);
   if (d.Ktot == 64) return launch_rw<2>(d, h, l, a_scale, os, st);
   return launch_rw<0>(d, h, l, a_scale, os, st);
diff --git a/edge-guided-near-eye-image-analysis-for-head-mounted-displays_amd/engine.py b/edge-guided-near-eye-image-analysis-for-head-mounted-displays_amd/engine.py
--- a/edge-guided-near-eye-image-analysis-for-head-mounted-displays_amd/engine.py
+++ b/edge-guided-near-eye-image-analysis-for-head-mounted-displays_amd/engine.py
@@ -148,6 +148,8 @@
 F16_STORAGE = os.environ.get("EGNE_F16_STORAGE", "1") != "0"
 F16_STORAGE_DEEP = os.environ.get("EGNE_F16_STORAGE_DEEP", "1") != "0"
 PRESPLIT_TRUNK = os.environ.get("EGNE_PRESPLIT_TRUNK", "1") != "0"
+PRESPLIT_STEM = min(int(os.environ.get("EGNE_PRESPLIT_STEM", "1")), 1)
+PRESPLIT_STEM_MIN_PIX = 1 << 18
 PRESPLIT = os.environ.get("EGNE_PRESPLIT", "1") != "0"
 SPLIT_PAIR_PERM = torch.tensor([16 * ((p >> 2) & 1) + 4 * (p >> 3) + (p & 3) for p in range(32)])
 
@@ -1192,9 +1194,15 @@
         if in3 is not None or out3 is not None:
             halo3 = (kind == "conv_f16x3:halo" and out3 is None and layer.dils[0] == 1
                      and layer.sfrag_coutp() == 32 and not cv.stats and cv.pool is None)
-            if not ((big or halo3) and not (big and choice.big1) and self.f16_products != 1 and calibrated and not self.train
-                    and p0.Cp % 32 == 0 and p0.off % 32 == 0 and (out3 is None or (int(d.Cout_store) % 32 == 0 and dst.off % 32 == 0))):
+            first3 = kind == "conv_f16x3:first" and in3 is None and layer.post is None
+            rw3 = (kind == "conv_f16x3:rw" and in3 is not None and p0.Cp >= 64 and layer.post is None and cv.residual is None and not cv.stats
+                   and (out3 is None or p0.Cp == 64)
+                   and (not choice.fused_pool or (out3 is not None and cv.pool.split3 is out3 and cv.pool.off % 32 == 0)))
+            if not ((big or halo3 or first3 or rw3) and not (big and choice.big1) and self.f16_products != 1 and calibrated and not self.train
+                    and (first3 or (p0.Cp % 32 == 0 and p0.off % 32 == 0)) and (out3 is None or (int(d.Cout_store) % 32 == 0 and dst.off % 32 == 0))):
                 raise NeedsFp32Storage(cv.name)
+        if cv.pool is not None and cv.pool.split3 is not out3:
+            raise NeedsFp32Storage(cv.name)
 
     def _calibration(self, cv):
         B, H, W = cv.B, cv.H, cv.W
@@ -1352,20 +1360,26 @@
             d.out_split, d.out_split_scale = 1, ps.value
             self.last_presplit = True
 
-            def cal_ps(args, vmax, d=d, layer=layer, ps=ps):
+            in3 = pieces[0].split3
+
+            def cal_ps(args, vmax, d=d, layer=layer, ps=ps, in3=in3):
+                if in3 is not None:
+                    vmax = getattr(in3, "vmax", None) or 2047.0 / in3.value
                 with torch.no_grad():
                     bound = vmax * float(layer.weights[0].detach().abs().sum(dim=(1, 2, 3)).max())
                     if layer.biases is not None and layer.biases[0] is not None:
                         bound += float(layer.biases[0].detach().abs().max())
                 ps.value = d.out_split_scale = _a_scale_for(bound)
-                return args[:3] + (_a_scale_for(vmax),) + args[4:]
-            cal3 = (cal_ps, list(pieces), B * H * W)
+                return args[:3] + (in3.value if in3 is not None else _a_scale_for(vmax),) + args[4:]
+            cal3 = (cal_ps, [], 0) if in3 is not None else (cal_ps, list(pieces), B * H * W)
         fin, fout = pieces[0].f16s, dst.f16s
         if fout is not None:
             assert not choice.fused_pool or pq.f16s is fout, "%s: the pooled second output shares the main output's storage scale" % name
             cal3 = self._f16_out(d, layer, dst, B * cv.Ho * cv.Wo, cal3, fin)
         if fin is not None:
             cal3 = self._f16_in(d, fin, cal3, 3)
+        if dst.split3 is not None:
+            self._split3_out([(len(self.calls), d)], dst, B * cv.Ho * cv.Wo)
         self._add(self.L.egne_conv3x3_rw_f16_fwd if rw else self.L.egne_conv3x3_rs_f16_fwd,
                   (C.byref(d), layer.fhi.data_ptr(), layer.flo.data_ptr(), F16X3_ASCALE, layer.w_scale), name, flops=cv.flops,
                   kind=choice.kind, cal=cal3, ws=[(4, layer, "w_scale")])
@@ -1405,6 +1419,8 @@
         d.CoutP = layer.c4_coutp
         if cv.dst.f16s is not None:
             cal3 = self._f16_out(d, layer, cv.dst, cv.B * cv.Ho * cv.Wo, cal3, None)
+        if cv.dst.split3 is not None:
+            self._split3_out([(len(self.calls), d)], cv.dst, cv.B * cv.Ho * cv.Wo)
         self._add(self.L.egne_conv3x3_smallcin_f16_fwd, (C.byref(d), layer.c4hi.data_ptr(), layer.c4lo.data_ptr(), F16X3_ASCALE,
                                                          layer.w_scale_c4), cv.name, flops=cv.flops, kind="conv_f16x3:first", cal=cal3, ws=[(4, layer, "w_scale_c4")])
 
```

After: 2209. No clear change (-0.4%).
